# hitfeelee/rtm3d

Measured on AMD Instinct MI355X. Metric: images_per_sec, higher is better.
Workload: dtype fp16

## Files before the change

rtm3d_amd/csrc/common.h:

```cpp
#pragma once
#include <hip/hip_runtime.h>
#include <stdint.h>
#include <stddef.h>

typedef _Float16 f16;
typedef _Float16 f16x8 __attribute__((ext_vector_type(8)));
typedef _Float16 f16x4 __attribute__((ext_vector_type(4)));
typedef _Float16 f16x2 __attribute__((ext_vector_type(2)));
typedef float f32x4 __attribute__((ext_vector_type(4)));
typedef uint32_t u32x4 __attribute__((ext_vector_type(4)));

__device__ __forceinline__ int div_small_q(int m, int d, float rcp_d) {
    const int q = (int)((float)m * rcp_d);
    const int r = m - q * d;
    return q + (r >= d ? 1 : 0) - (r < 0 ? 1 : 0);
}


#define RT_DMA16(gptr, lds_byte_addr) \
    asm volatile("s_mov_b32 m0, %1\n\ts_nop 0\n\tglobal_load_lds_dwordx4 %0, off" : : "v"(gptr), "s"(lds_byte_addr) : "memory", "m0")
#define RT_DMA16_NT(gptr, lds_byte_addr) \
    asm volatile("s_mov_b32 m0, %1\n\ts_nop 0\n\tglobal_load_lds_dwordx4 %0, off nt" : : "v"(gptr), "s"(lds_byte_addr) : "memory", "m0")
static __device__ __forceinline__ const void* rt_uniform_ptr(const void* p) {
    const unsigned long long v = (unsigned long long)p;
    const unsigned lo = (unsigned)__builtin_amdgcn_readfirstlane((int)(unsigned)v), hi = (unsigned)__builtin_amdgcn_readfirstlane((int)(unsigned)(v >> 32));
    return (const void*)(((unsigned long long)hi << 32) | lo);
}
#define RT_DMA16_SBASE(voff_bytes, sbase, lds_byte_addr) \
    asm volatile("s_mov_b32 m0, %2\n\ts_nop 0\n\tglobal_load_lds_dwordx4 %0, %1" : : "v"(voff_bytes), "s"(rt_uniform_ptr(sbase)), "s"(lds_byte_addr) : "memory", "m0")

#define RT_DMA16_SBASE_LANES(voff_bytes, sbase, lds_byte_addr, lanemask) \
    { unsigned long long rt_exec_; \
      asm volatile("s_mov_b64 %0, exec\n\ts_and_b64 exec, exec, %4\n\ts_mov_b32 m0, %3\n\ts_nop 0\n\tglobal_load_lds_dwordx4 %1, %2\n\ts_mov_b64 exec, %0" \
                   : "=&s"(rt_exec_) : "v"(voff_bytes), "s"(rt_uniform_ptr(sbase)), "s"(lds_byte_addr), "s"(lanemask) : "memory", "m0", "scc"); }
#define RT_DMA16_SBASE_NT(voff_bytes, sbase, lds_byte_addr) \
    asm volatile("s_mov_b32 m0, %2\n\ts_nop 0\n\tglobal_load_lds_dwordx4 %0, %1 nt" : : "v"(voff_bytes), "s"(rt_uniform_ptr(sbase)), "s"(lds_byte_addr) : "memory", "m0")

#define RT_MAX_GROUPS 4
#define RT_MAX_TAPS 80

struct ConvGroupArgs {
    int in_coff, out_coff, res_coff;
    int out_oy, out_ox;
    uint32_t w_off;
    int bias_off;
    int tap_off[RT_MAX_TAPS];
};

struct ConvKArgs {
    const f16* in;
    const f16* wgt;
    const float* bias;
    const f16* res;
    void* out;
    int M, HmWm, Wm;
    int in_Hp, in_Wp, in_C, in_stride, in_P;
    int out_Hp, out_Wp, out_C, out_scale, out_P;
    int res_Hp, res_Wp, res_C, res_P;
    int cin, cout, ksteps, cpt;
    int ntaps;
    int relu, MT, NT;
    int out_H, out_W;
    float* slab;
    int ksplit;
    int deep;
    f16* s2d;
    int s_Hp, s_Wp, s_C, s_P, s_coff;
    int in_s2d;
    ConvGroupArgs g[RT_MAX_GROUPS];
};

struct HaloTaps { unsigned long long taps[RT_MAX_GROUPS]; };

struct PoolKArgs {
    const f16* in; f16* out;
    int B, Ho, Wo, C8;
    int in_Hp, in_Wp, in_C, in_P, in_coff;
    int out_Hp, out_Wp, out_C, out_P, out_coff;
    int ksize, stride, pad;
};

struct SoftmaxKArgs {
    const f16* z_in; f16* z_out;
    const f16* u[3];
    int n_u;
    int B, H, W, C;
    int z_Hp, z_Wp, z_C, z_P;
    int zi_Hp, zi_Wp, zi_C, zi_P;
    int u_Hp[3], u_Wp[3], u_C[3], u_P[3];
    float* partial;
    float* stats;
    int chunks, rows_per_chunk;
    int apply_chunks, apply_rows, xsplit, seg_w;
    int partial_chunks;
};

__device__ __forceinline__ int xcd_contiguous_index(int b, int n) {
#ifdef RT_TIMING_NO_XCD_ORDER
    return b;
#endif
    const int q = n >> 3, r = n & 7, xcd = b & 7, k = b >> 3;
    return xcd * q + (xcd < r ? xcd : r) + k;
}

struct HeadOutArgs {
    const f16* in;
    const f16* wgt;
    const float* bias;
    float* out[4];
    int cout[4];
    int nheads;
    int B, H, W;
    int in_Hp, in_Wp, in_C, in_P;
    int tiles_x, tiles_y, tile_rows;
};

struct StemFusedArgs {
    const f16* x4;
    const float* x_nchw;
    f16* out;
    const f16* w_base;
    const f16* w_l0;
    const f16* w_l1;
    const float* b_base;
    const float* b_l0;
    const float* b_l1;
    int B, H, W;
    int x_Hp, x_Wp, x_P;
    int o_Hp, o_Wp, o_C, o_P, o_coff;
    int tiles_x, tiles_y;
};

struct Conv32S2Args {
    const f16* in;
    f16* out_conv;
    f16* out_proj;
    const f16* w_conv;
    const f16* w_proj;
    const float* b_conv;
    const float* b_proj;
    int B, Ho, Wo;
    int in_Hp, in_Wp, in_C, in_P, in_coff;
    int oc_Hp, oc_Wp, oc_C, oc_P, oc_coff;
    int op_Hp, op_Wp, op_C, op_P, op_coff;
};

struct RootKArgs {
    const f16* w;
    const float* bias;
    f16* out;
    int o_Hp, o_Wp, o_C, o_P, o_coff;
    f16* pool;
    int p_Hp, p_Wp, p_C, p_P, p_coff;
    f16* s2d;
    int s_Hp, s_Wp, s_C, s_P, s_coff;
    int relu;
};

struct PatchMaskArgs {
    f16* base;
    const int32_t* yx;
    int n_slots, S, C, img_H, img_W, origin;
};

struct ConvMx8Args {
    const uint8_t* in; const uint8_t* in_s;
    const uint8_t* wgt;
    const uint8_t* wsc;
    const float* bias;
    void* out; uint8_t* out_s;
    int M, HmWm, Wm;
    int in_Hp, in_Wp, in_C, in_P;
    int out_Hp, out_Wp, out_C, out_P;
    int cin, cout, ntaps, cpt, ksteps;
    int relu, out_fp16, MT, NT;
    int in_coff[RT_MAX_GROUPS], out_coff[RT_MAX_GROUPS];
    int tap_pix[RT_MAX_TAPS];
};
struct QuantMx8Args {
    const f16* in;
    uint8_t* out;
    uint8_t* out_s;
    int B, H, W;
    int in_Hp, in_Wp, in_C, in_P, in_coff;
    int out_Hp, out_Wp, out_C, out_P, out_coff;
    int nblk;
};

struct PersistentGrid { int grid, single; };
inline PersistentGrid persistent_grid(int total, int cu_count) { return {cu_count < total ? cu_count : total, total <= cu_count ? 1 : 0}; }

hipError_t launch_patch_mask(const PatchMaskArgs& a, hipStream_t s);
hipError_t launch_conv32s2_fused(const Conv32S2Args& a, int cu_count, unsigned int* ticket_ctr, hipStream_t s);
hipError_t launch_stem_fused(const StemFusedArgs& a, hipStream_t s);
hipError_t launch_conv_headout(const HeadOutArgs& a, hipStream_t s);
hipError_t launch_conv_mfma(const ConvKArgs& a, int bn_tile, int groups, int epi_nchw, hipStream_t s);
hipError_t launch_conv_mfma_deep(const ConvKArgs& a, int bn_tile, int groups, unsigned int* tile_ctr, hipStream_t s);
hipError_t launch_conv_mfma256(const ConvKArgs& a, int groups, unsigned int* tile_ctr, float* stat_out, hipStream_t s);
enum Conv256Route { C256_ONE_TILE, C256_PERSISTENT, C256_HALO, C256_LATTICE };
Conv256Route conv_mfma256_route(const ConvKArgs& a, int groups, HaloTaps* ht);
void conv_mfma256_permute_weights(const f16* src, f16* dst, size_t n_ktiles);
bool conv64_halo_supported(const ConvKArgs& a, int groups);
hipError_t launch_conv64_halo(const ConvKArgs& a, int cu_count, unsigned int* ticket_ctr, hipStream_t s);
hipError_t launch_conv64_root(const ConvKArgs& a, const RootKArgs& r, int cu_count, unsigned int* ticket_ctr, hipStream_t s);
bool conv64s2_halo_supported(const ConvKArgs& a, int groups);
hipError_t launch_conv64s2_halo(const ConvKArgs& a, int cu_count, unsigned int* ticket_ctr, hipStream_t s);
bool conv128_halo_supported(const ConvKArgs& a, int groups);
hipError_t launch_conv128_halo(const ConvKArgs& a, int cu_count, unsigned int* ticket_ctr, hipStream_t s);
hipError_t launch_conv_smallc(const ConvKArgs& a, hipStream_t s);
bool conv_smallc_supported(int cin, int cout, int ntaps);
hipError_t launch_nchw_to_nhwc4(const float* in, f16* out, int B, int H, int W, int Hp, int Wp, int P, hipStream_t s);
hipError_t launch_maxpool(const PoolKArgs& a, hipStream_t s);
hipError_t launch_softmax_fuse(const SoftmaxKArgs& a, hipStream_t s);
hipError_t launch_quant_mx8(const QuantMx8Args& a, hipStream_t s);
hipError_t launch_conv_mx8(const ConvMx8Args& a, int groups, hipStream_t s);
```

rtm3d_amd/csrc/conv_mfma256.hip:

```cpp
#include <string.h>
#include "common.h"

#define LDS_AS __attribute__((address_space(3)))
#define GLB_AS __attribute__((address_space(1)))

void conv_mfma256_permute_weights(const f16* src, f16* dst, size_t n_ktiles) {
    for (size_t k = 0; k < n_ktiles; ++k)
        for (int rd = 0; rd < 256; ++rd) {
            const int j = rd >> 7, wc = (rd >> 5) & 3, c = (rd >> 4) & 1, frow = rd & 15;
            const int rs = wc * 64 + frow * 4 + j * 2 + c;
            for (int pos = 0; pos < 8; ++pos) {
                const int chunk = pos ^ (rd & 7);
                memcpy(dst + (k * 256 + rd) * 64 + pos * 8, src + (k * 256 + rs) * 64 + (chunk ^ (rs & 7)) * 8, 16);
            }
        }
}

#define HALF_ELEMS (128 * 64)
#define BUF_ELEMS (4 * HALF_ELEMS)
#define SLOT_XA 0
#define SLOT_XB 1
#define SLOT_WA 2
#define SLOT_WB 3

__device__ __forceinline__ void c256_next_pixel(int& n, int& y, int& x, bool live, int Wm, int Hm) {
    const bool wx = x + 1 == Wm, wy = wx && y + 1 == Hm;
    const int x1 = wx ? 0 : x + 1, y1 = wy ? 0 : (wx ? y + 1 : y), n1 = wy ? n + 1 : n;
    x = live ? x1 : x; y = live ? y1 : y; n = live ? n1 : n;
}

template <int RES>
__global__ __launch_bounds__(512) void conv_mfma256_kernel(const ConvKArgs a) {
    __shared__ __attribute__((aligned(16))) f16 lds[2 * BUF_ELEMS + HALF_ELEMS];
    const int tid = threadIdx.x;
    const int lane = tid & 63;
    const int wave = __builtin_amdgcn_readfirstlane(tid >> 6);
    const int wp = wave & 1, wc = wave >> 1;

    const int bid = blockIdx.x;
    const int xcd = bid & 7, jb = bid >> 3;
    const int chunk = (a.MT + 7) >> 3;
    const int ntile = jb % a.NT;
    const int mtile = xcd * chunk + jb / a.NT;
    if (mtile >= a.MT) return;
    const ConvGroupArgs& g = a.g[blockIdx.y];
    const int T = a.ksteps;

    uint32_t xoff[2][2];
    {
        const int rr = tid >> 3, cs = tid & 7;
#pragma unroll
        for (int h = 0; h < 2; ++h)
#pragma unroll
            for (int i = 0; i < 2; ++i) {
                int m = mtile * 256 + h * 128 + i * 64 + rr;
                m = m < a.M ? m : a.M - 1;
                const int n = m / a.HmWm, rem = m - n * a.HmWm;
                const int y = rem / a.Wm, x = rem - y * a.Wm;
                const uint32_t pix = (uint32_t)((n * a.in_Hp + y * a.in_stride + a.in_P) * a.in_Wp + x * a.in_stride + a.in_P);
                xoff[h][i] = pix * (uint32_t)a.in_C + (uint32_t)g.in_coff + (uint32_t)((cs ^ (rr & 7)) * 8);
            }
    }
    const f16* wbase = a.wgt + g.w_off + (size_t)ntile * T * (256 * 64);
    f16* const dummy = lds + 2 * BUF_ELEMS;

    auto stage = [&](int slot, int kt) {
        const bool live = kt < T;
        const int k = live ? kt : T - 1;
        f16* dst = live ? (lds + (k & 1) * BUF_ELEMS + slot * HALF_ELEMS) : dummy;
        if (slot < 2) {
            const int tap = k / a.cpt, q = k - tap * a.cpt;
            const int koff = g.tap_off[tap] + q * 64;
#pragma unroll
            for (int i = 0; i < 2; ++i) {
                const f16* src = a.in + (size_t)xoff[slot][i] + (ptrdiff_t)koff;
                __builtin_amdgcn_global_load_lds((const GLB_AS void*)src, (LDS_AS void*)(dst + (i * 512 + wave * 64) * 8), 16, 0, 0);
            }
        } else {
            const f16* ws = wbase + (size_t)k * (256 * 64) + (slot - 2) * HALF_ELEMS;
#pragma unroll
            for (int i = 0; i < 2; ++i)
                __builtin_amdgcn_global_load_lds((const GLB_AS void*)(ws + (i * 512 + tid) * 8),
                                                 (LDS_AS void*)(dst + (i * 512 + wave * 64) * 8), 16, 0, 0);
        }
    };

    f32x4 acc[2][2][2][4];
#pragma unroll
    for (int i = 0; i < 2; ++i)
#pragma unroll
        for (int j = 0; j < 2; ++j)
#pragma unroll
            for (int c = 0; c < 2; ++c)
#pragma unroll
                for (int p = 0; p < 4; ++p) acc[i][j][c][p] = (f32x4){0.f, 0.f, 0.f, 0.f};

    const int frow = lane & 15, fk = lane >> 4;
    const int sw0 = ((0 * 4 + fk) ^ (frow & 7)) * 8, sw1 = ((1 * 4 + fk) ^ (frow & 7)) * 8;
    const int xrow = (wp * 64 + frow) * 64;
    const int wrow = (wc * 32 + frow) * 64;

    stage(SLOT_XA, 0); stage(SLOT_WA, 0); stage(SLOT_WB, 0); stage(SLOT_XB, 0);
    stage(SLOT_XA, 1); stage(SLOT_WA, 1);
    asm volatile("s_waitcnt vmcnt(4)" ::: "memory");
    __builtin_amdgcn_s_barrier();
    if (wave >= 4) __builtin_amdgcn_s_barrier();

    f16x8 xf[4][2], wa[2][2], wb[2][2];

#define LOAD_X(slot_base)                                                                   \
    _Pragma("unroll") for (int p = 0; p < 4; ++p) {                                         \
        xf[p][0] = *(const f16x8*)((slot_base) + xrow + p * 1024 + sw0);                    \
        xf[p][1] = *(const f16x8*)((slot_base) + xrow + p * 1024 + sw1);                    \
    }
#define LOAD_W(dstf, slot_base)                                                             \
    _Pragma("unroll") for (int c = 0; c < 2; ++c) {                                         \
        dstf[c][0] = *(const f16x8*)((slot_base) + wrow + c * 1024 + sw0);                  \
        dstf[c][1] = *(const f16x8*)((slot_base) + wrow + c * 1024 + sw1);                  \
    }
#define SEG_SYNC()                                                                          \
    asm volatile("s_waitcnt vmcnt(8)" ::: "memory");                                        \
    __builtin_amdgcn_sched_barrier(0);                                                      \
    __builtin_amdgcn_s_barrier();                                                           \
    __builtin_amdgcn_sched_barrier(0);
#define MMA(i, j, wfrag)                                                                    \
    __builtin_amdgcn_s_setprio(1);                                                          \
    _Pragma("unroll") for (int kk = 0; kk < 2; ++kk)                                        \
        _Pragma("unroll") for (int c = 0; c < 2; ++c)                                       \
            _Pragma("unroll") for (int p = 0; p < 4; ++p)                                   \
                acc[i][j][c][p] = __builtin_amdgcn_mfma_f32_16x16x32_f16(xf[p][kk], wfrag[c][kk], acc[i][j][c][p], 0, 0, 0); \
    __builtin_amdgcn_s_setprio(0);                                                          \
    __builtin_amdgcn_sched_barrier(0);                                                      \
    __builtin_amdgcn_s_barrier();                                                           \
    __builtin_amdgcn_sched_barrier(0);

    for (int t = 0; t < T; ++t) {
        const f16* buf = lds + (t & 1) * BUF_ELEMS;
        LOAD_X(buf + SLOT_XA * HALF_ELEMS)
        LOAD_W(wa, buf + SLOT_WA * HALF_ELEMS)
        stage(SLOT_WB, t + 1);
        SEG_SYNC()
        MMA(0, 0, wa)
        LOAD_W(wb, buf + SLOT_WB * HALF_ELEMS)
        stage(SLOT_XB, t + 1);
        SEG_SYNC()
        MMA(0, 1, wb)
        LOAD_X(buf + SLOT_XB * HALF_ELEMS)
        stage(SLOT_XA, t + 2);
        SEG_SYNC()
        MMA(1, 1, wb)
        stage(SLOT_WA, t + 2);
        SEG_SYNC()
        MMA(1, 0, wa)
    }
    if (wave < 4) __builtin_amdgcn_s_barrier();

    const f32x4 bv = *(const f32x4*)(a.bias + g.bias_off + ntile * 256 + wc * 64 + frow * 4);
    const float lo = a.relu ? 0.f : -__builtin_inff();
    const int cbase = ntile * 256 + wc * 64 + frow * 4;
    const int Hm = a.HmWm / a.Wm;
#pragma unroll
    for (int i = 0; i < 2; ++i) {
        size_t opix[4][4];
        f16x4 rv[4][4];
#pragma unroll
        for (int p = 0; p < 4; ++p) {
            const int m0 = mtile * 256 + i * 128 + wp * 64 + p * 16 + fk * 4;
            const int m = m0 < a.M ? m0 : a.M - 1;
            int n = m / a.HmWm;
            const int rem = m - n * a.HmWm;
            int y = rem / a.Wm, x = rem - y * a.Wm;
#pragma unroll
            for (int e = 0; e < 4; ++e) {
                if (e) c256_next_pixel(n, y, x, m0 + e < a.M, a.Wm, Hm);
                const int oy = y * a.out_scale + g.out_oy, ox = x * a.out_scale + g.out_ox;
                opix[p][e] = ((size_t)(n * a.out_Hp + oy + a.out_P) * a.out_Wp + ox + a.out_P) * a.out_C + g.out_coff + cbase;
                if (RES) rv[p][e] = *(const f16x4*)(a.res + ((size_t)(n * a.res_Hp + oy + a.res_P) * a.res_Wp + ox + a.res_P) * a.res_C + g.res_coff + cbase);
            }
        }
#pragma unroll
        for (int p = 0; p < 4; ++p)
#pragma unroll
            for (int e = 0; e < 4; ++e) {
                f32x4 v = {acc[i][0][0][p][e], acc[i][0][1][p][e], acc[i][1][0][p][e], acc[i][1][1][p][e]};
                v += bv;
                if (RES) {
                    const f16x4 r = rv[p][e];
                    v[0] += (float)r[0]; v[1] += (float)r[1]; v[2] += (float)r[2]; v[3] += (float)r[3];
                }
                const f16x4 h = {(f16)fmaxf(v[0], lo), (f16)fmaxf(v[1], lo), (f16)fmaxf(v[2], lo), (f16)fmaxf(v[3], lo)};
                *(f16x4*)((f16*)a.out + opix[p][e]) = h;
            }
    }
}

#define CONV256_MAX_BIAS 2048
#define DMA16 RT_DMA16
#define DMA16_NT RT_DMA16_NT
#define DMA16_SBASE RT_DMA16_SBASE
#define DMA16_SBASE_NT RT_DMA16_SBASE_NT
#define LDS_F16X8(byte_addr) (*(const LDS_AS f16x8*)(uintptr_t)(byte_addr))
#define LOAD_X_N(SLOT)                                                                      \
    _Pragma("unroll") for (int p = 0; p < 4; ++p) {                                         \
        xf[p][0] = LDS_F16X8(xaddr0 + (SLOT) * HALF_ELEMS * 2 + p * 2048);                  \
        xf[p][1] = LDS_F16X8(xaddr1 + (SLOT) * HALF_ELEMS * 2 + p * 2048);                  \
    }
#define LOAD_W_N(dstf, SLOT)                                                                \
    _Pragma("unroll") for (int c = 0; c < 2; ++c) {                                         \
        dstf[c][0] = LDS_F16X8(waddr0 + (SLOT) * HALF_ELEMS * 2 + c * 2048);                \
        dstf[c][1] = LDS_F16X8(waddr1 + (SLOT) * HALF_ELEMS * 2 + c * 2048);                \
    }
#ifdef C256_T_NOVM
#define SEG_SYNC_N(VM)                                                                      \
    asm volatile("s_waitcnt lgkmcnt(0)" ::: "memory");                                      \
    __builtin_amdgcn_sched_barrier(0);                                                      \
    __builtin_amdgcn_s_barrier();                                                           \
    __builtin_amdgcn_sched_barrier(0);
#else
#define SEG_SYNC_N(VM)                                                                      \
    asm volatile("s_waitcnt vmcnt(" #VM ") lgkmcnt(0)" ::: "memory");                       \
    __builtin_amdgcn_sched_barrier(0);                                                      \
    __builtin_amdgcn_s_barrier();                                                           \
    __builtin_amdgcn_sched_barrier(0);
#endif
#define MMA_N(i, j, wfrag, FIRST, TAILBAR)                                                  \
    __builtin_amdgcn_s_setprio(1);                                                          \
    _Pragma("unroll") for (int kk = 0; kk < 2; ++kk)                                        \
        _Pragma("unroll") for (int c = 0; c < 2; ++c)                                       \
            _Pragma("unroll") for (int p = 0; p < 4; ++p)                                   \
                acc[i][j][c][p] = __builtin_amdgcn_mfma_f32_16x16x32_f16(xf[p][kk], wfrag[c][kk], acc[i][j][c][p], 0, 0, 0); \
    __builtin_amdgcn_s_setprio(0);                                                          \
    __builtin_amdgcn_sched_barrier(0);                                                      \
    if (TAILBAR) __builtin_amdgcn_s_barrier();                                              \
    __builtin_amdgcn_sched_barrier(0);
#ifdef C256_STAMPS
#define C256_STAMP_KT 20
#define C256_STAMP_N 20
#define STAMP(k) if ((wave & 3) == 0 && stamp_tile == 1 && t < C256_STAMP_KT) { unsigned long long ts_; \
        asm volatile("s_memtime %0\n\ts_waitcnt lgkmcnt(0)" : "=s"(ts_) :: "memory"); if (lane == 0) lds_stamp[wave >> 2][t][k] = ts_; }
#define TSTAMP(k) if ((wave & 3) == 0 && stamp_tile < 4) { unsigned long long ts_; \
        asm volatile("s_memtime %0\n\ts_waitcnt lgkmcnt(0)" : "=s"(ts_) :: "memory"); if (lane == 0) lds_tstamp[wave >> 2][stamp_tile][k] = ts_; }
#else
#define STAMP(k)
#define TSTAMP(k)
#endif
#ifdef C256_STAMPS
#define SEG_SYNC_S(VM, K0)                                                                  \
    STAMP((K0) + 0)                                                                         \
    asm volatile("s_waitcnt vmcnt(" #VM ") lgkmcnt(0)" ::: "memory");                       \
    STAMP((K0) + 1)                                                                         \
    __builtin_amdgcn_sched_barrier(0);                                                      \
    __builtin_amdgcn_s_barrier();                                                           \
    __builtin_amdgcn_sched_barrier(0);                                                      \
    STAMP((K0) + 2)
#define MMA_S(i, j, wfrag, FIRST, TAILBAR, K0)                                              \
    __builtin_amdgcn_s_setprio(1);                                                          \
    _Pragma("unroll") for (int kk = 0; kk < 2; ++kk)                                        \
        _Pragma("unroll") for (int c = 0; c < 2; ++c)                                       \
            _Pragma("unroll") for (int p = 0; p < 4; ++p)                                   \
                acc[i][j][c][p] = __builtin_amdgcn_mfma_f32_16x16x32_f16(xf[p][kk], wfrag[c][kk], acc[i][j][c][p], 0, 0, 0); \
    __builtin_amdgcn_s_setprio(0);                                                          \
    __builtin_amdgcn_sched_barrier(0);                                                      \
    STAMP((K0) + 3)                                                                         \
    if (TAILBAR) __builtin_amdgcn_s_barrier();                                              \
    __builtin_amdgcn_sched_barrier(0);                                                      \
    STAMP((K0) + 4)
#else
#define SEG_SYNC_S(VM, K0) SEG_SYNC_N(VM)
#define MMA_S(i, j, wfrag, FIRST, TAILBAR, K0) MMA_N(i, j, wfrag, FIRST, TAILBAR)
#endif
#if !defined(C256_WB_IN_P4)
#define STAGE_WB_P1 stage_w1(SLOT_WB, 0, t + 1, sp ^ 1);
#define STAGE_WB_P2 stage_w1(SLOT_WB, 1, t + 1, sp ^ 1);
#define STAGE_WB_P4
#define VM1_8 5
#define VM1_40 37
#else
#define STAGE_WB_P1
#define STAGE_WB_P2
#define STAGE_WB_P4 stage(SLOT_WB, t + 2, sp, 0);
#define VM1_8 8
#define VM1_40 40
#endif
#define OPA_SET(SP)                                                                         \
    {                                                                                       \
        const uint32_t bufb_ = lds_base + (uint32_t)(SP) * (BUF_ELEMS * 2);                 \
        opa[0] = bufb_ + xrow_b0; opa[1] = bufb_ + xrow_b1; opa[2] = bufb_ + wrow_b0; opa[3] = bufb_ + wrow_b1; \
    }
#define STEP_N(VM, VM1, FIRST, LAST)                                                          \
    {                                                                                       \
         \
        const uint32_t xaddr0 = opa[0], xaddr1 = opa[1], waddr0 = opa[2], waddr1 = opa[3];  \
        LOAD_X_N(SLOT_XA)                                                                   \
        LOAD_W_N(wa, SLOT_WA)                                                               \
        STAGE_WB_P1                                                                         \
        SEG_SYNC_S(VM1, 0)                                                                  \
        MMA_S(0, 0, wa, FIRST, 1, 0)                                                        \
        LOAD_W_N(wb, SLOT_WB)                                                               \
        stage(SLOT_XB, t + 1, sp ^ 1, koff1);                                               \
        STAGE_WB_P2                                                                         \
        SEG_SYNC_S(VM, 5)                                                                   \
        MMA_S(0, 1, wb, FIRST, 1, 5)                                                        \
        LOAD_X_N(SLOT_XB)                                                                   \
        stage(SLOT_XA, t + 2, sp, koff2);                                                   \
        SEG_SYNC_S(VM, 10)                                                                  \
        MMA_S(1, 1, wb, FIRST, 1, 10)                                                       \
         \
              \
        int kchan3;                                                                         \
        int kraw3 = koff_parts(t + 3, kchan3);                                              \
        stage(SLOT_WA, t + 2, sp, 0);                                                       \
        OPA_SET(sp ^ 1)                                                                     \
        asm volatile("" : "+v"(opa[0]), "+v"(opa[1]), "+v"(opa[2]), "+v"(opa[3]));          \
        STAGE_WB_P4                                                                         \
        SEG_SYNC_S(VM, 15)                                                                  \
        asm volatile("" : "+s"(kraw3));            \
        const int koff3 = kraw3 + kchan3;                                                   \
        MMA_S(1, 0, wa, FIRST, !(LAST), 15)                                                 \
        koff1 = koff2; koff2 = koff3;                                                       \
        sp ^= 1;                                                                            \
    }

template <int RES, int XNT>
__global__ __launch_bounds__(512) void conv_mfma256_persistent_kernel(const ConvKArgs a, const int groups, const int nbias, unsigned int* tile_ctr, const int one_list) {
    __shared__ __attribute__((aligned(16))) f16 lds[2 * BUF_ELEMS + HALF_ELEMS];
    __shared__ __attribute__((aligned(16))) float lds_bias[CONV256_MAX_BIAS + 4];
#ifdef C256_STAMPS
    __shared__ unsigned long long lds_stamp[2][C256_STAMP_KT][C256_STAMP_N];
    __shared__ unsigned long long lds_tstamp[2][4][4];
    int stamp_tile = 0;
#endif
    const int tid = threadIdx.x;
    const int lane = tid & 63;
    const int wave = __builtin_amdgcn_readfirstlane(tid >> 6);
    const int wp = wave & 1, wc = wave >> 1;
    const int T = a.ksteps;
    for (int i = tid; i < nbias; i += 512) lds_bias[i] = a.bias[i];
    __syncthreads();

    const int xcd = one_list ? 0 : blockIdx.x & 7, per_xcd = one_list ? gridDim.x : gridDim.x >> 3;
    const int chunk = one_list ? a.MT : (a.MT + 7) >> 3;
    int mt_here = a.MT - xcd * chunk;
    mt_here = mt_here < 0 ? 0 : (mt_here > chunk ? chunk : mt_here);
    const int jbs = mt_here * a.NT;
    const int vtotal = jbs * groups;
    int* const lds_ticket = (int*)(lds_bias + CONV256_MAX_BIAS);
    const int last_draw = vtotal + per_xcd - 1;
    if (tid == 0) {
        const int t0 = (int)atomicAdd(&tile_ctr[xcd], 1u);
        if (t0 == last_draw) tile_ctr[xcd] = 0u;
        lds_ticket[0] = t0;
    }
    __syncthreads();
    const int v = __builtin_amdgcn_readfirstlane(lds_ticket[0]);
    if (v >= vtotal) return;

    const uint32_t lds_base = (uint32_t)(uintptr_t)(LDS_AS f16*)lds;
    const int rr = tid >> 3, cs = tid & 7;
    const float rcp_hw = 1.0f / (float)a.HmWm, rcp_w = 1.0f / (float)a.Wm;
    uint32_t xo_c[2][2], xo_n[2][2];
    const f16 *wb_c, *wb_n;
    int gi_c, gi_n, mt_c, mt_n, nt_c, nt_n;
    auto locate = [&](int vv, uint32_t (&xo)[2][2], const f16*& wb, int& gi, int& mt, int& nt) {
        gi = vv / jbs;
        const int jb = vv - gi * jbs;
        const int q = jb / a.NT;
        nt = jb - q * a.NT;
        mt = xcd * chunk + q;
        const ConvGroupArgs& g = a.g[gi];
#pragma unroll
        for (int h = 0; h < 2; ++h)
#pragma unroll
            for (int i = 0; i < 2; ++i) {
                int m = mt * 256 + h * 128 + i * 64 + rr;
                m = m < a.M ? m : a.M - 1;
                const int n = div_small_q(m, a.HmWm, rcp_hw), rem = m - n * a.HmWm;
                const int y = div_small_q(rem, a.Wm, rcp_w), x = rem - y * a.Wm;
                const uint32_t pix = (uint32_t)((n * a.in_Hp + y * a.in_stride + a.in_P) * a.in_Wp + x * a.in_stride + a.in_P);
                xo[h][i] = (pix * (uint32_t)a.in_C + (uint32_t)g.in_coff + (uint32_t)((cs ^ (rr & 7)) * 8)) * 2u;
            }
#ifdef C256_T_WSAME
        wb = a.wgt + g.w_off;
#else
        wb = a.wgt + g.w_off + (size_t)nt * T * (256 * 64);
#endif
    };
    bool live_n;
    locate(v, xo_c, wb_c, gi_c, mt_c, nt_c);
    xo_n[0][0] = xo_c[0][0]; xo_n[0][1] = xo_c[0][1]; xo_n[1][0] = xo_c[1][0]; xo_n[1][1] = xo_c[1][1];
    wb_n = wb_c; gi_n = gi_c; mt_n = mt_c; nt_n = nt_c; live_n = false;

    auto koff_parts = [&](int kpos, int& chan) -> int {
        const bool in_cur = kpos < T;
        const int k = in_cur ? kpos : kpos - T;
        const int tap = k / a.cpt;
        chan = (k - tap * a.cpt) * 64;
        return a.g[in_cur ? gi_c : gi_n].tap_off[tap];
    };
    auto koff_of = [&](int kpos) -> int { int c; const int r = koff_parts(kpos, c); return r + c; };
    const uint32_t wvoff = (uint32_t)tid * 16u;
    auto stage_w1 = [&](int slot, int i, int kpos, int par) {
        const bool in_cur = kpos < T;
        const int k = in_cur ? kpos : kpos - T;
        const uint32_t dst0 = lds_base + (uint32_t)((in_cur || live_n) ? par * BUF_ELEMS + slot * HALF_ELEMS : 2 * BUF_ELEMS) * 2u;
        const f16* ws = (in_cur ? wb_c : wb_n) + (size_t)k * (256 * 64) + (slot - 2) * HALF_ELEMS;
        DMA16_SBASE(wvoff, ws + i * 512 * 8, __builtin_amdgcn_readfirstlane(dst0 + (uint32_t)((i * 512 + wave * 64) * 16)));
    };
    auto stage = [&](int slot, int kpos, int par, int koff) {
        const bool in_cur = kpos < T;
        const int k = in_cur ? kpos : kpos - T;
        const uint32_t dst0 = lds_base + (uint32_t)((in_cur || live_n) ? par * BUF_ELEMS + slot * HALF_ELEMS : 2 * BUF_ELEMS) * 2u;
        if (slot < 2) {
#ifdef C256_T_NOX
            return;
#endif
            const f16* xbase = a.in + (ptrdiff_t)koff;
#pragma unroll
            for (int i = 0; i < 2; ++i) {
                const uint32_t xo = in_cur ? xo_c[slot][i] : xo_n[slot][i];
                if (XNT) DMA16_SBASE_NT(xo, xbase, __builtin_amdgcn_readfirstlane(dst0 + (uint32_t)((i * 512 + wave * 64) * 16)));
                else DMA16_SBASE(xo, xbase, __builtin_amdgcn_readfirstlane(dst0 + (uint32_t)((i * 512 + wave * 64) * 16)));
            }
        } else {
#ifdef C256_T_NOW
            return;
#endif
            const f16* ws = (in_cur ? wb_c : wb_n) + (size_t)k * (256 * 64) + (slot - 2) * HALF_ELEMS;
#pragma unroll
            for (int i = 0; i < 2; ++i)
                DMA16_SBASE(wvoff, ws + i * 512 * 8, __builtin_amdgcn_readfirstlane(dst0 + (uint32_t)((i * 512 + wave * 64) * 16)));
        }
    };

    f32x4 acc[2][2][2][4];
    const int frow = lane & 15, fk = lane >> 4;
    const int sw0 = ((0 * 4 + fk) ^ (frow & 7)) * 8, sw1 = ((1 * 4 + fk) ^ (frow & 7)) * 8;
    const uint32_t xrow_b0 = (uint32_t)(((wp * 64 + frow) * 64 + sw0) * 2), xrow_b1 = (uint32_t)(((wp * 64 + frow) * 64 + sw1) * 2);
    const uint32_t wrow_b0 = (uint32_t)(((wc * 32 + frow) * 64 + sw0) * 2), wrow_b1 = (uint32_t)(((wc * 32 + frow) * 64 + sw1) * 2);
    const int Hm = a.HmWm / a.Wm;
    const f16 lo = a.relu ? (f16)0.f : (f16)(-__builtin_inff());
    const f16x4 lo4 = {lo, lo, lo, lo};

    stage(SLOT_XA, 0, 0, koff_of(0)); stage(SLOT_WA, 0, 0, 0); stage(SLOT_WB, 0, 0, 0); stage(SLOT_XB, 0, 0, koff_of(0));
    stage(SLOT_XA, 1, 1, koff_of(1)); stage(SLOT_WA, 1, 1, 0);
#ifndef C256_WB_IN_P4
    asm volatile("s_waitcnt vmcnt(4)" ::: "memory");
#else
    stage(SLOT_WB, 1, 1, 0);
    asm volatile("s_waitcnt vmcnt(6)" ::: "memory");
#endif
    if (tid == 0) {
        const int t1 = (int)atomicAdd(&tile_ctr[xcd], 1u);
        if (t1 == last_draw) tile_ctr[xcd] = 0u;
        lds_ticket[1] = t1;
    }
    asm volatile("s_waitcnt lgkmcnt(0)" ::: "memory");
    __builtin_amdgcn_s_barrier();
    int vnext = __builtin_amdgcn_readfirstlane(lds_ticket[1]);
    if (wave >= 4) __builtin_amdgcn_s_barrier();

    f16x8 xf[4][2], wa[2][2], wb[2][2];
    int sp = 0;
    int tpar = 0;
    int koff1 = koff_of(1), koff2 = koff_of(2);
    bool first_tile = true;
    uint32_t opa[4];
    OPA_SET(0)

    for (;;) {
        int ticket = vnext;
        const bool draw = vnext < vtotal;
        if (wave == 0 && draw) {
            const unsigned inc = 1u, off = (unsigned)xcd * 4u;
            unsigned long long saved_exec;
            asm volatile("s_mov_b64 %1, exec\n\ts_mov_b64 exec, 1\n\tglobal_atomic_add %0, %2, %3, %4 sc0\n\ts_mov_b64 exec, %1"
                         : "=&v"(ticket), "=&s"(saved_exec) : "v"(off), "v"(inc), "s"(tile_ctr) : "memory");
        }
        {
            f32x4 b4 = *(const f32x4*)__builtin_assume_aligned(lds_bias + a.g[gi_c].bias_off + nt_c * 256 + wc * 64 + frow * 4, 16);
            asm volatile("" : "+v"(b4));
#pragma unroll
            for (int j = 0; j < 2; ++j)
#pragma unroll
                for (int c = 0; c < 2; ++c) {
                    const float b = b4[j * 2 + c];
#pragma unroll
                    for (int i = 0; i < 2; ++i)
#pragma unroll
                        for (int p = 0; p < 4; ++p) acc[i][j][c][p] = (f32x4){b, b, b, b};
                }
        }
        int t = 0;
        TSTAMP(0)
        if (first_tile) STEP_N(8, VM1_8, 1, 0) else STEP_N(40, VM1_40, 1, 0)
        first_tile = false;
        if (wave == 0) {
            asm volatile("s_waitcnt vmcnt(8)" : "+v"(ticket) : : "memory");
            if (lane == 0) {
                lds_ticket[tpar] = ticket;
                if (draw && ticket == last_draw) tile_ctr[xcd] = 0u;
            }
        }
        live_n = draw;
        if (live_n) locate(vnext, xo_n, wb_n, gi_n, mt_n, nt_n);
        for (t = 1; t < T - 1; ++t) STEP_N(8, VM1_8, 0, 0)
        STEP_N(8, VM1_8, 0, 1)
        if (wave < 4) __builtin_amdgcn_s_barrier();
        TSTAMP(1)

        {
            const ConvGroupArgs& g = a.g[gi_c];
            const int cbase = nt_c * 256 + wc * 64 + frow * 4;
#pragma unroll
            for (int i = 0; i < 2; ++i) {
                size_t opix[4][4];
                f16x4 rv[4][4];
#pragma unroll
                for (int p = 0; p < 4; ++p) {
                    const int m0 = mt_c * 256 + i * 128 + wp * 64 + p * 16 + fk * 4;
                    const int m = m0 < a.M ? m0 : a.M - 1;
                    int n = div_small_q(m, a.HmWm, rcp_hw);
                    const int rem = m - n * a.HmWm;
                    int y = div_small_q(rem, a.Wm, rcp_w), x = rem - y * a.Wm;
#pragma unroll
                    for (int e = 0; e < 4; ++e) {
                        if (e) c256_next_pixel(n, y, x, m0 + e < a.M, a.Wm, Hm);
                        const int oy = y * a.out_scale + g.out_oy, ox = x * a.out_scale + g.out_ox;
                        opix[p][e] = ((size_t)(n * a.out_Hp + oy + a.out_P) * a.out_Wp + ox + a.out_P) * a.out_C + g.out_coff + cbase;
                        if (RES) rv[p][e] = *(const f16x4*)(a.res + ((size_t)(n * a.res_Hp + oy + a.res_P) * a.res_Wp + ox + a.res_P) * a.res_C + g.res_coff + cbase);
                    }
                }
#pragma unroll
                for (int p = 0; p < 4; ++p)
#pragma unroll
                    for (int e = 0; e < 4; ++e) {
                        f32x4 vv = {acc[i][0][0][p][e], acc[i][0][1][p][e], acc[i][1][0][p][e], acc[i][1][1][p][e]};
                        if (RES) {
                            const f16x4 r = rv[p][e];
                            vv[0] += (float)r[0]; vv[1] += (float)r[1]; vv[2] += (float)r[2]; vv[3] += (float)r[3];
                        }
                        f16x4 h = {(f16)vv[0], (f16)vv[1], (f16)vv[2], (f16)vv[3]};
                        h = __builtin_elementwise_max(h, lo4);
                        *(f16x4*)((f16*)a.out + opix[p][e]) = h;
                    }
            }
        }
        TSTAMP(2)
        if (wave >= 4) __builtin_amdgcn_s_barrier();
        TSTAMP(3)
#ifdef C256_STAMPS
        ++stamp_tile;
#endif
        if (!live_n) break;
        vnext = __builtin_amdgcn_readfirstlane(lds_ticket[tpar]);
        tpar ^= 1;
        xo_c[0][0] = xo_n[0][0]; xo_c[0][1] = xo_n[0][1]; xo_c[1][0] = xo_n[1][0]; xo_c[1][1] = xo_n[1][1];
        wb_c = wb_n; gi_c = gi_n; mt_c = mt_n; nt_c = nt_n;
    }
    if (wave < 4) __builtin_amdgcn_s_barrier();
#ifdef C256_STAMPS
    if ((blockIdx.x == 0 || blockIdx.x == 101) && (wave & 3) == 0) {
        asm volatile("s_waitcnt vmcnt(0) lgkmcnt(0)" ::: "memory");
        unsigned long long* dst = (unsigned long long*)(tile_ctr + 1024) + (blockIdx.x ? 1 : 0) * 1024 + (wave >> 2) * 512;
        for (int i = lane; i < C256_STAMP_KT * C256_STAMP_N; i += 64) dst[i] = (&lds_stamp[wave >> 2][0][0])[i];
        if (lane < 16) dst[C256_STAMP_KT * C256_STAMP_N + lane] = (&lds_tstamp[wave >> 2][0][0])[lane];
        if (lane == 16) dst[C256_STAMP_KT * C256_STAMP_N + 16] = (unsigned long long)T;
    }
#endif
}

bool conv_mfma256_halo_supported(const ConvKArgs& a, int groups, HaloTaps* ht);
hipError_t launch_conv_mfma256_halo(const ConvKArgs& a, const HaloTaps& ht, int groups, int nbias, int cu_count, unsigned int* tile_ctr, float* stat_out, hipStream_t s);
int conv_mfma256_lattice_dilation(const ConvKArgs& a, int groups);
hipError_t launch_conv_mfma256_lattice(const ConvKArgs& a, int groups, int nbias, int cu_count, unsigned int* tile_ctr, hipStream_t s);

static int device_cu_count() {
    static int n = 0;
    if (!n) {
        int dev = 0;
        hipDeviceProp_t prop;
        if (hipGetDevice(&dev) != hipSuccess || hipGetDeviceProperties(&prop, dev) != hipSuccess) return 256;
        n = prop.multiProcessorCount;
    }
    return n;
}

static int conv256_nbias(const ConvKArgs& a, int groups) {
    int nbias = 0;
    for (int g = 0; g < groups; ++g) nbias = a.g[g].bias_off + a.cout > nbias ? a.g[g].bias_off + a.cout : nbias;
    return (nbias + 255) / 256 * 256;
}

Conv256Route conv_mfma256_route(const ConvKArgs& a, int groups, HaloTaps* ht) {
    const int nbias = conv256_nbias(a, groups);
    const unsigned long long in_bytes = (unsigned long long)(a.M / a.HmWm) * a.in_Hp * a.in_Wp * a.in_C * 2ull;
    if (a.ksteps < 4 || nbias > CONV256_MAX_BIAS || in_bytes >= (1ull << 32)) return C256_ONE_TILE;
    HaloTaps scratch;
    if (!ht) ht = &scratch;
#ifdef C256_T_NOHALO9
    if (a.ntaps == 9) {} else
#endif
    if (!a.res && (a.ntaps == 9 || a.ntaps == 4) && nbias <= 1024 && conv_mfma256_halo_supported(a, groups, ht)) return C256_HALO;
#ifndef C256_T_NOLATTICE
    if (nbias <= 1024 && conv_mfma256_lattice_dilation(a, groups) != 0) return C256_LATTICE;
#endif
    return C256_PERSISTENT;
}

hipError_t launch_conv_mfma256(const ConvKArgs& a, int groups, unsigned int* tile_ctr, float* stat_out, hipStream_t s) {
    dim3 block(512, 1, 1);
    HaloTaps ht;
    const Conv256Route route = conv_mfma256_route(a, groups, &ht);
    if (stat_out && route != C256_HALO) return hipErrorInvalidValue;
    if (route != C256_ONE_TILE && !tile_ctr) return hipErrorInvalidValue;
    const int nbias = conv256_nbias(a, groups);
    if (route == C256_HALO) return launch_conv_mfma256_halo(a, ht, groups, nbias, device_cu_count(), tile_ctr, stat_out, s);
    if (route == C256_LATTICE) return launch_conv_mfma256_lattice(a, groups, nbias, device_cu_count(), tile_ctr, s);
    if (route == C256_PERSISTENT) {
        const int per_xcd = device_cu_count() / 8;
        const int one_list = (long long)a.MT * a.NT * groups <= device_cu_count() ? 1 : 0;
        dim3 grid(per_xcd * 8, 1, 1);
        const bool x_once = !a.res && a.ntaps == 1 && a.NT == 1 && a.in_stride == 1;
        if (a.res) hipLaunchKernelGGL((conv_mfma256_persistent_kernel<1, 0>), grid, block, 0, s, a, groups, nbias, tile_ctr, one_list);
        else if (x_once) hipLaunchKernelGGL((conv_mfma256_persistent_kernel<0, 1>), grid, block, 0, s, a, groups, nbias, tile_ctr, one_list);
        else hipLaunchKernelGGL((conv_mfma256_persistent_kernel<0, 0>), grid, block, 0, s, a, groups, nbias, tile_ctr, one_list);
        return hipGetLastError();
    }
    const int mt8 = (a.MT + 7) / 8 * 8;
    dim3 grid(mt8 * a.NT, groups, 1);
    if (a.res) hipLaunchKernelGGL((conv_mfma256_kernel<1>), grid, block, 0, s, a);
    else hipLaunchKernelGGL((conv_mfma256_kernel<0>), grid, block, 0, s, a);
    return hipGetLastError();
}
```

rtm3d_amd/csrc/pool_softmax.hip:

```cpp
#include "common.h"

__global__ __launch_bounds__(256) void maxpool_kernel(const PoolKArgs a) {
    const int idx = blockIdx.x * 256 + threadIdx.x;
    const int total = a.B * a.Ho * a.Wo * a.C8;
    if (idx >= total) return;
    const int c8 = idx % a.C8;
    int p = idx / a.C8;
    const int ox = p % a.Wo; p /= a.Wo;
    const int oy = p % a.Ho;
    const int n = p / a.Ho;
    f16x8 m;
    bool first = true;
    if (a.ksize == 0) {
        const f16* ip = a.in + ((size_t)(n * a.in_Hp + oy + a.in_P) * a.in_Wp + ox + a.in_P) * a.in_C + a.in_coff + c8 * 8;
        m = *(const f16x8*)ip;
#pragma unroll
        for (int ph = 1; ph < 4; ++ph) {
            const f16x8 v = *(const f16x8*)(ip + ph * a.C8 * 8);
#pragma unroll
            for (int e = 0; e < 8; ++e) m[e] = v[e] > m[e] ? v[e] : m[e];
        }
        first = false;
    }
    for (int ky = 0; ky < a.ksize; ++ky)
        for (int kx = 0; kx < a.ksize; ++kx) {
            const int iy = oy * a.stride - a.pad + ky + a.in_P, ix = ox * a.stride - a.pad + kx + a.in_P;
            const f16x8 v = *(const f16x8*)(a.in + ((size_t)(n * a.in_Hp + iy) * a.in_Wp + ix) * a.in_C + a.in_coff + c8 * 8);
            if (first) { m = v; first = false; }
            else {
#pragma unroll
                for (int e = 0; e < 8; ++e) m[e] = v[e] > m[e] ? v[e] : m[e];
            }
        }
    *(f16x8*)(a.out + ((size_t)(n * a.out_Hp + oy + a.out_P) * a.out_Wp + ox + a.out_P) * a.out_C + a.out_coff + c8 * 8) = m;
}

hipError_t launch_maxpool(const PoolKArgs& a, hipStream_t s) {
    const int total = a.B * a.Ho * a.Wo * a.C8;
    hipLaunchKernelGGL(maxpool_kernel, dim3((total + 255) / 256), dim3(256), 0, s, a);
    return hipGetLastError();
}

__global__ __launch_bounds__(256) void softmax_reduce_kernel(const SoftmaxKArgs a) {
    const int chunk = blockIdx.x, n = blockIdx.y, ui = blockIdx.z;
    const int lane = threadIdx.x & 63, wave = threadIdx.x >> 6;
    const int cg = lane & 31, slot = wave * 2 + (lane >> 5);
    const f16* u = a.u[ui];
    const int Hp = a.u_Hp[ui], Wp = a.u_Wp[ui], C = a.u_C[ui], P = a.u_P[ui];
    float m[8], s[8];
#pragma unroll
    for (int e = 0; e < 8; ++e) { m[e] = -INFINITY; s[e] = 0.f; }
    const int y0 = chunk * a.rows_per_chunk;
    const int y1 = min(y0 + a.rows_per_chunk, a.H);
    for (int y = y0; y < y1; ++y) {
        const f16* row = u + ((size_t)(n * Hp + y + P) * Wp + P) * C + cg * 8;
        for (int x = slot; x < a.W; x += 32) {
            f16x8 v[4];
#pragma unroll
            for (int k = 0; k < 4; ++k) {
                const int xx = x + 8 * k < a.W ? x + 8 * k : x;
                v[k] = *(const f16x8*)(row + (size_t)xx * C);
            }
#pragma unroll
            for (int e = 0; e < 8; ++e) {
                float f[4];
#pragma unroll
                for (int k = 0; k < 4; ++k) f[k] = (x + 8 * k < a.W) ? (float)v[k][e] : -INFINITY;
                const float mn = fmaxf(fmaxf(fmaxf(f[0], f[1]), fmaxf(f[2], f[3])), m[e]);
                s[e] = s[e] * __expf(m[e] - mn) + ((__expf(f[0] - mn) + __expf(f[1] - mn)) + (__expf(f[2] - mn) + __expf(f[3] - mn)));
                m[e] = mn;
            }
        }
    }
    __shared__ float sm[8][256], ss[8][256];
#pragma unroll
    for (int e = 0; e < 8; ++e) { sm[slot][cg * 8 + e] = m[e]; ss[slot][cg * 8 + e] = s[e]; }
    __syncthreads();
    const int c = threadIdx.x;
    float M = -INFINITY;
#pragma unroll
    for (int w = 0; w < 8; ++w) M = fmaxf(M, sm[w][c]);
    float S = 0.f;
#pragma unroll
    for (int w = 0; w < 8; ++w) S += (sm[w][c] == -INFINITY) ? 0.f : ss[w][c] * __expf(sm[w][c] - M);
    float* out = a.partial + ((((size_t)ui * a.B + n) * a.chunks + chunk) * a.C + c) * 2;
    out[0] = M; out[1] = S;
}

__global__ __launch_bounds__(1024) void softmax_combine_kernel(const SoftmaxKArgs a) {
    const int n = blockIdx.x, ui = blockIdx.y, cl = threadIdx.x & 63, c = blockIdx.z * 64 + cl, part = threadIdx.x >> 6;
    const int chunks = a.partial_chunks > 0 ? a.partial_chunks : a.chunks;
    const float2* p = (const float2*)a.partial + ((size_t)ui * a.B + n) * chunks * a.C + c;
    float m = -INFINITY, sum = 0.f;
    for (int k = part; k < chunks; k += 16) {
        const float2 v = p[(size_t)k * a.C];
        if (v.x != -INFINITY) {
            const float mn = fmaxf(m, v.x);
            sum = sum * __expf(m - mn) + v.y * __expf(v.x - mn);
            m = mn;
        }
    }
    __shared__ float sm[16][64], ss[16][64];
    sm[part][cl] = m; ss[part][cl] = sum;
    __syncthreads();
    if (part == 0) {
        float mm = sm[0][cl];
#pragma unroll
        for (int w = 1; w < 16; ++w) mm = fmaxf(mm, sm[w][cl]);
        float t = 0.f;
#pragma unroll
        for (int w = 0; w < 16; ++w) t += (sm[w][cl] == -INFINITY) ? 0.f : ss[w][cl] * __expf(sm[w][cl] - mm);
        float* o = a.stats + (((size_t)ui * a.B + n) * a.C + c) * 2;
        o[0] = mm; o[1] = 1.f / t;
    }
}

template <int NU>
__global__ __launch_bounds__(256) void softmax_apply_kernel(const SoftmaxKArgs a) {
    const int chunk = blockIdx.x, n = blockIdx.y;
    const int rchunk = chunk / a.xsplit, xseg = chunk - rchunk * a.xsplit;
    const int x0 = xseg * a.seg_w, x1 = min(x0 + a.seg_w, a.W);
    const int lane = threadIdx.x & 63, wave = threadIdx.x >> 6;
    const int cg = lane & 31, slot = wave * 2 + (lane >> 5);
    float M[NU][8], invS[NU][8];
#pragma unroll
    for (int ui = 0; ui < NU; ++ui) {
        const float* st = a.stats + (((size_t)ui * a.B + n) * a.C + cg * 8) * 2;
#pragma unroll
        for (int e = 0; e < 8; ++e) { M[ui][e] = st[2 * e]; invS[ui][e] = st[2 * e + 1]; }
    }
    const int y0 = rchunk * a.apply_rows;
    const int y1 = min(y0 + a.apply_rows, a.H);
    for (int y = y0; y < y1; ++y) {
        const size_t zrow = ((size_t)(n * a.z_Hp + y + a.z_P) * a.z_Wp + a.z_P) * a.z_C + cg * 8;
        const size_t zirow = ((size_t)(n * a.zi_Hp + y + a.zi_P) * a.zi_Wp + a.zi_P) * a.zi_C + cg * 8;
        size_t urow[NU];
#pragma unroll
        for (int ui = 0; ui < NU; ++ui) urow[ui] = ((size_t)(n * a.u_Hp[ui] + y + a.u_P[ui]) * a.u_Wp[ui] + a.u_P[ui]) * a.u_C[ui] + cg * 8;
        for (int x = x0 + slot; x < x1; x += 16) {
            f16x8 zi[2], v[2][NU];
#pragma unroll
            for (int k = 0; k < 2; ++k) {
                const int xx = x + 8 * k < x1 ? x + 8 * k : x;
                zi[k] = __builtin_nontemporal_load((const f16x8*)(a.z_in + zirow + (size_t)xx * a.zi_C));
#pragma unroll
                for (int ui = 0; ui < NU; ++ui) v[k][ui] = __builtin_nontemporal_load((const f16x8*)(a.u[ui] + urow[ui] + (size_t)xx * a.u_C[ui]));
            }
#pragma unroll
            for (int k = 0; k < 2; ++k) {
                if (x + 8 * k >= x1) break;
                f16x8 o;
#pragma unroll
                for (int e = 0; e < 8; ++e) {
                    float acc = (float)zi[k][e];
#pragma unroll
                    for (int ui = 0; ui < NU; ++ui) {
                        const float f = (float)v[k][ui][e];
                        acc += f * (__expf(f - M[ui][e]) * invS[ui][e]);
                    }
                    o[e] = (f16)acc;
                }
                *(f16x8*)(a.z_out + zrow + (size_t)(x + 8 * k) * a.z_C) = o;
            }
        }
    }
}

hipError_t launch_softmax_fuse(const SoftmaxKArgs& a, hipStream_t s) {
    if (a.C != 256 || a.n_u < 1 || a.n_u > 3 || a.xsplit < 1 || a.seg_w < 1 || a.apply_rows < 1) return hipErrorInvalidValue;
    if (a.partial_chunks <= 0) hipLaunchKernelGGL(softmax_reduce_kernel, dim3(a.chunks, a.B, a.n_u), dim3(256), 0, s, a);
    hipLaunchKernelGGL(softmax_combine_kernel, dim3(a.B, a.n_u, a.C / 64), dim3(1024), 0, s, a);
    if (a.n_u == 3) hipLaunchKernelGGL(softmax_apply_kernel<3>, dim3(a.apply_chunks, a.B, 1), dim3(256), 0, s, a);
    else if (a.n_u == 2) hipLaunchKernelGGL(softmax_apply_kernel<2>, dim3(a.apply_chunks, a.B, 1), dim3(256), 0, s, a);
    else hipLaunchKernelGGL(softmax_apply_kernel<1>, dim3(a.apply_chunks, a.B, 1), dim3(256), 0, s, a);
    return hipGetLastError();
}
```

rtm3d_amd/csrc/runtime.hip:

```cpp
#include <math.h>
#include <stdarg.h>
#include <stdio.h>
#include <string.h>
#include <string>
#include <vector>

#include "common.h"
#include "../../include/rtm3d_hip.h"

static thread_local char g_err[512] = "";
void rt_set_error(const char* fmt, ...) {
    va_list ap;
    va_start(ap, fmt);
    vsnprintf(g_err, sizeof(g_err), fmt, ap);
    va_end(ap);
}
#define RT_FAIL(...) do { rt_set_error(__VA_ARGS__); return 1; } while (0)
#define RT_HIP(expr) do { hipError_t e_ = (expr); if (e_ != hipSuccess) { rt_set_error("%s: %s", #expr, hipGetErrorString(e_)); return 1; } } while (0)

struct Tensor {
    int B, H, W, C, P, Hp, Wp;
    f16* alloc;
    f16* base;
    size_t elems;
};

struct MxTensor {
    int B, H, W, C, P, Hp, Wp;
    uint8_t* alloc;
    uint8_t* base;
    uint8_t* s_alloc;
    uint8_t* s_base;
    size_t elems;
};

enum OpKind { OP_CONV_MFMA, OP_CONV_MFMA256, OP_CONV64_HALO, OP_CONV64_ROOT, OP_CONV64S2_HALO, OP_CONV128_HALO, OP_STEM_FUSED, OP_CONV32S2_FUSED, OP_CONV_SMALLC, OP_INPUT4, OP_HEADOUT, OP_MAXPOOL, OP_SOFTMAX, OP_PATCH_MASK, OP_QUANT_MX8, OP_CONV_MX8 };

struct Op {
    OpKind kind;
    std::string name;
    double flops, bytes;
    ConvKArgs conv; int groups, bn_tile, epi_nchw, out_slot;
    int ticket_slot = -1;
    float* stat_out = nullptr;
    Tensor input4;
    bool input4_unread = false;
    PoolKArgs pool;
    SoftmaxKArgs sm;
    HeadOutArgs ho;
    StemFusedArgs sf;
    Conv32S2Args c32;
    PatchMaskArgs pm;
    RootKArgs root;
    QuantMx8Args qm;
    ConvMx8Args cm;
};

struct rtm3d_ctx {
    int device;
    int n_cus = 256;
    std::vector<Tensor> tensors;
    std::vector<struct MxTensor> mx8;
    std::vector<void*> blobs;
    std::vector<size_t> blob_bytes;
    std::vector<Op> ops;
    std::vector<void*> extra;
    float* stat_buf = nullptr;
    int stat_chunks = 0, stat_B = 0;
    int stat_tensor[3] = {-1, -1, -1};
    unsigned int* tile_ctr = nullptr;
    int ticket_slots_used = 0;
    float* slab = nullptr;
    size_t slab_floats = 0;
    int probe_op = -1;
    std::vector<hipEvent_t> probe_ev;
    int probe_count = 0;
    int graph_mode = 0;
    hipStream_t capture_stream = nullptr;
    hipStream_t last_stream = nullptr;
    bool has_last = false;
    hipEvent_t done_ev = nullptr;
    struct GraphEntry { const void* key[5]; hipGraph_t graph; hipGraphExec_t exec; unsigned long long last_use; };
    std::vector<GraphEntry> graphs;
    unsigned long long graph_clock = 0, graph_hits = 0, graph_captures = 0, graph_refused = 0;
    int test_memset_in_replay = 0;
    int n_marks = 0;
    int mark_op[8];
    hipEvent_t mark_ev[9];
    void* engine = nullptr;
    void (*engine_free)(void*) = nullptr;
};

void rt_ctx_attach_engine(rtm3d_ctx* ctx, void* engine, void (*engine_free)(void*)) {
    ctx->engine = engine;
    ctx->engine_free = engine_free;
}
void* rt_ctx_engine(rtm3d_ctx* ctx) { return ctx ? ctx->engine : nullptr; }

static const int PROBE_RING = 64;
static const int TICKET_SLOTS = 56;
static const int SPLIT_CTRS = 256;
static const size_t TILE_CTR_WORDS = 8 + TICKET_SLOTS + SPLIT_CTRS;
static const size_t DEBUG_WORD0 = 1024;
static const size_t DEBUG_WORDS = 16384;

static int ensure_tile_ctr(rtm3d_ctx* ctx) {
    if (ctx->tile_ctr) return 0;
    RT_HIP(hipMalloc((void**)&ctx->tile_ctr, (DEBUG_WORD0 + DEBUG_WORDS) * sizeof(unsigned int)));
    RT_HIP(hipMemset(ctx->tile_ctr, 0, (DEBUG_WORD0 + DEBUG_WORDS) * sizeof(unsigned int)));
    ctx->extra.push_back(ctx->tile_ctr);
    return 0;
}
static unsigned int* ticket_ctr(rtm3d_ctx* ctx, const Op& op) { return ctx->tile_ctr + 8 + op.ticket_slot; }
static unsigned int* split_ctrs(rtm3d_ctx* ctx) { return ctx->tile_ctr + 8 + TICKET_SLOTS; }

static int claim_ticket(rtm3d_ctx* ctx, Op& op, const char* what) {
    if (ctx->ticket_slots_used >= TICKET_SLOTS) RT_FAIL("%s: out of ticket counters", what);
    if (ensure_tile_ctr(ctx)) return 1;
    op.ticket_slot = ctx->ticket_slots_used++;
    return 0;
}

static bool slice_ok(int coff, int n, int C) { return coff >= 0 && coff + n <= C && coff % 8 == 0; }

extern "C" const char* rtm3d_last_error(void) { return g_err; }
extern "C" int rtm3d_abi_version(void) { return RTM3D_ABI_VERSION; }

extern "C" int rtm3d_ctx_create(int device, rtm3d_ctx** out) {
    if (!out) RT_FAIL("ctx_create: null out");
    RT_HIP(hipSetDevice(device));
    int xccs = 0, cus = 0;
    RT_HIP(hipDeviceGetAttribute(&cus, hipDeviceAttributeMultiprocessorCount, device));
    if (hipDeviceGetAttribute(&xccs, hipDeviceAttributeNumberOfXccs, device) != hipSuccess) xccs = 0;
    if ((xccs != 0 && xccs != 8) || cus < 8 || (cus % 8) != 0)
        RT_FAIL("ctx_create: device %d reports %d XCCs / %d CUs; librtm3d_hip is built for the 8-XCD (SPX) MI355X", device, xccs, cus);
    rtm3d_ctx* c = new rtm3d_ctx();
    c->device = device;
    c->n_cus = cus;
    *out = c;
    return 0;
}

extern "C" void rtm3d_ctx_destroy(rtm3d_ctx* ctx) {
    if (!ctx) return;
    for (auto& t : ctx->tensors) (void)hipFree(t.alloc);
    for (auto& t : ctx->mx8) { (void)hipFree(t.alloc); (void)hipFree(t.s_alloc); }
    for (auto p : ctx->blobs) (void)hipFree(p);
    for (auto p : ctx->extra) (void)hipFree(p);
    for (auto e : ctx->probe_ev) (void)hipEventDestroy(e);
    for (auto& ge : ctx->graphs) { (void)hipGraphExecDestroy(ge.exec); (void)hipGraphDestroy(ge.graph); }
    if (ctx->capture_stream) (void)hipStreamDestroy(ctx->capture_stream);
    if (ctx->done_ev) (void)hipEventDestroy(ctx->done_ev);
    if (ctx->engine_free) ctx->engine_free(ctx->engine);
    delete ctx;
}

static const size_t GUARD = 4096;

extern "C" int rtm3d_tensor_create(rtm3d_ctx* ctx, int B, int H, int W, int C, int pad, int* id) {
    if (!ctx || !id) RT_FAIL("tensor_create: null argument");
    if (B <= 0 || H <= 0 || W <= 0 || C <= 0 || pad < 0 || (C % 4) != 0) RT_FAIL("tensor_create: bad shape B=%d H=%d W=%d C=%d pad=%d (C must be a multiple of 4)", B, H, W, C, pad);
    Tensor t;
    t.B = B; t.H = H; t.W = W; t.C = C; t.P = pad; t.Hp = H + 2 * pad; t.Wp = W + 2 * pad;
    t.elems = (size_t)B * t.Hp * t.Wp * C;
    if (t.elems >= ((size_t)1 << 32) - 2 * GUARD) RT_FAIL("tensor_create: %zu elements exceed the 32-bit offset range of the kernels", t.elems);
    const size_t bytes = (t.elems + 2 * GUARD) * sizeof(f16);
    RT_HIP(hipMalloc((void**)&t.alloc, bytes));
    RT_HIP(hipMemset(t.alloc, 0, bytes));
    t.base = t.alloc + GUARD;
    ctx->tensors.push_back(t);
    *id = (int)ctx->tensors.size() - 1;
    return 0;
}

static Tensor* get_tensor(rtm3d_ctx* ctx, int id) {
    if (id < 0 || id >= (int)ctx->tensors.size()) return nullptr;
    return &ctx->tensors[id];
}

extern "C" int rtm3d_tensor_download(rtm3d_ctx* ctx, int id, int c0, int C, float* h_nchw) {
    Tensor* t = ctx ? get_tensor(ctx, id) : nullptr;
    if (!t || !h_nchw || c0 < 0 || C <= 0 || c0 + C > t->C) RT_FAIL("tensor_download: bad arguments");
    std::vector<f16> host(t->elems);
    RT_HIP(hipDeviceSynchronize());
    RT_HIP(hipMemcpy(host.data(), t->base, t->elems * sizeof(f16), hipMemcpyDeviceToHost));
    for (int n = 0; n < t->B; ++n)
        for (int c = 0; c < C; ++c)
            for (int y = 0; y < t->H; ++y)
                for (int x = 0; x < t->W; ++x)
                    h_nchw[(((size_t)n * C + c) * t->H + y) * t->W + x] =
                        (float)host[(((size_t)n * t->Hp + y + t->P) * t->Wp + x + t->P) * t->C + c0 + c];
    return 0;
}

extern "C" int rtm3d_tensor_upload(rtm3d_ctx* ctx, int id, int c0, int C, const float* h_nchw) {
    Tensor* t = ctx ? get_tensor(ctx, id) : nullptr;
    if (!t || !h_nchw || c0 < 0 || C <= 0 || c0 + C > t->C) RT_FAIL("tensor_upload: bad arguments");
    std::vector<f16> host(t->elems);
    RT_HIP(hipDeviceSynchronize());
    RT_HIP(hipMemcpy(host.data(), t->base, t->elems * sizeof(f16), hipMemcpyDeviceToHost));
    for (int n = 0; n < t->B; ++n)
        for (int c = 0; c < C; ++c)
            for (int y = 0; y < t->H; ++y)
                for (int x = 0; x < t->W; ++x)
                    host[(((size_t)n * t->Hp + y + t->P) * t->Wp + x + t->P) * t->C + c0 + c] =
                        (f16)h_nchw[(((size_t)n * C + c) * t->H + y) * t->W + x];
    RT_HIP(hipMemcpy(t->base, host.data(), t->elems * sizeof(f16), hipMemcpyHostToDevice));
    return 0;
}

extern "C" int rtm3d_blob_create(rtm3d_ctx* ctx, const void* h_data, size_t bytes, int* id) {
    if (!ctx || !h_data || !id || bytes == 0) RT_FAIL("blob_create: bad arguments");
    void* p = nullptr;
    RT_HIP(hipMalloc(&p, bytes + 256));
    RT_HIP(hipMemset(p, 0, bytes + 256));
    RT_HIP(hipMemcpy(p, h_data, bytes, hipMemcpyHostToDevice));
    ctx->blobs.push_back(p);
    ctx->blob_bytes.push_back(bytes);
    *id = (int)ctx->blobs.size() - 1;
    return 0;
}

extern "C" int rtm3d_tensor_info(rtm3d_ctx* ctx, int id, void** d_base, int* B, int* H, int* W, int* C, int* border) {
    Tensor* t = ctx ? get_tensor(ctx, id) : nullptr;
    if (!t) RT_FAIL("tensor_info: bad tensor %d", id);
    if (d_base) *d_base = t->base;
    if (B) *B = t->B;
    if (H) *H = t->H;
    if (W) *W = t->W;
    if (C) *C = t->C;
    if (border) *border = t->P;
    return 0;
}

static void* get_blob(rtm3d_ctx* ctx, int id, size_t* bytes);
extern "C" int rtm3d_blob_address(rtm3d_ctx* ctx, int id, void** d_ptr, size_t* bytes) {
    void* p = ctx ? get_blob(ctx, id, bytes) : nullptr;
    if (!p || !d_ptr) RT_FAIL("blob_address: bad blob %d", id);
    *d_ptr = p;
    return 0;
}

static void* get_blob(rtm3d_ctx* ctx, int id, size_t* bytes) {
    if (id < 0 || id >= (int)ctx->blobs.size()) return nullptr;
    if (bytes) *bytes = ctx->blob_bytes[id];
    return ctx->blobs[id];
}

static int admit_mfma128(rtm3d_ctx* ctx, const rtm3d_conv_desc* d, size_t wbytes, size_t bbytes, Op& op) {
    ConvKArgs& a = op.conv;
    const int BN = d->bn_tile;
    if (BN != 16 && BN != 32 && BN != 64 && BN != 128) RT_FAIL("op_conv: bn_tile must be 16/32/64/128");
    if (d->cin % 64) RT_FAIL("op_conv(mfma): cin=%d is not a multiple of 64", d->cin);
    if (!d->out_nchw_f32 && (d->cout % BN)) RT_FAIL("op_conv(mfma): cout=%d is not a multiple of the tile %d", d->cout, BN);
    if (d->out_nchw_f32 && a.res) RT_FAIL("op_conv(mfma): the NCHW fp32 epilogue adds no residual");
    const int cout_pad = (d->cout + BN - 1) / BN * BN;
    a.cpt = d->cin / 64; a.ksteps = d->ntaps * a.cpt;
    a.MT = (a.M + 127) / 128; a.NT = cout_pad / BN;
    const size_t per_group = (size_t)cout_pad * a.ksteps * 64;
    if (wbytes != per_group * d->groups * sizeof(f16)) RT_FAIL("op_conv(mfma): packed weight blob has %zu bytes, expected %zu", wbytes, per_group * d->groups * sizeof(f16));
    if (bbytes != (size_t)cout_pad * d->groups * sizeof(float)) RT_FAIL("op_conv(mfma): bias blob has %zu bytes, expected %zu", bbytes, (size_t)cout_pad * d->groups * sizeof(float));
    for (int g = 0; g < d->groups; ++g) { a.g[g].w_off = (uint32_t)(per_group * g); a.g[g].bias_off = cout_pad * g; }
    op.kind = OP_CONV_MFMA; op.bn_tile = BN;
    op.name = d->ntaps == 1 ? "conv1x1_mfma" : (d->ntaps == 4 ? "deconv4x4_phase_mfma" : "conv3x3_mfma");
    if (d->out_nchw_f32 || (BN != 64 && BN != 128)) return 0;
    const long long wgs = (long long)a.MT * a.NT * d->groups;
    if (wgs > ctx->n_cus) return 0;
    a.deep = 1;
    op.name += "_deep";
    if (ensure_tile_ctr(ctx)) return 1;
    if (wgs * 2 > ctx->n_cus || wgs > SPLIT_CTRS || a.ksteps < 8) return 0;
    int ks = (int)(ctx->n_cus / wgs);
    if (ks > a.ksteps / 4) ks = a.ksteps / 4;
    if (ks > 16) ks = 16;
    if (ks < 2) return 0;
    const size_t need = (size_t)ks * wgs * 128 * BN;
    if (need > ctx->slab_floats) {
        float* nslab = nullptr;
        RT_HIP(hipMalloc((void**)&nslab, need * sizeof(float)));
        ctx->extra.push_back(nslab);
        for (auto& prev : ctx->ops) if (prev.kind == OP_CONV_MFMA && prev.conv.ksplit > 1) prev.conv.slab = nslab;
        ctx->slab = nslab; ctx->slab_floats = need;
    }
    a.ksplit = ks; a.slab = ctx->slab;
    op.name += "_splitk";
    return 0;
}

static int admit_mfma256(rtm3d_ctx* ctx, const rtm3d_conv_desc* d, size_t wbytes, size_t bbytes, Op& op) {
    ConvKArgs& a = op.conv;
    if (d->cin % 64 || d->cout % 256 || d->out_nchw_f32) RT_FAIL("op_conv(mfma256): needs cin %% 64 == 0, cout %% 256 == 0, NHWC output (cin=%d cout=%d)", d->cin, d->cout);
    a.cpt = d->cin / 64; a.ksteps = d->ntaps * a.cpt;
    a.MT = (a.M + 255) / 256; a.NT = d->cout / 256;
    const size_t per_group = (size_t)d->cout * a.ksteps * 64;
    if (wbytes != per_group * d->groups * sizeof(f16)) RT_FAIL("op_conv(mfma256): packed weight blob has %zu bytes, expected %zu", wbytes, per_group * d->groups * sizeof(f16));
    if (bbytes != (size_t)d->cout * d->groups * sizeof(float)) RT_FAIL("op_conv(mfma256): bias blob size mismatch");
    for (int g = 0; g < d->groups; ++g) { a.g[g].w_off = (uint32_t)(per_group * g); a.g[g].bias_off = d->cout * g; }
    op.kind = OP_CONV_MFMA256; op.bn_tile = 256;
    if (ensure_tile_ctr(ctx)) return 1;
    {
        std::vector<f16> h_src(wbytes / sizeof(f16)), h_dst(wbytes / sizeof(f16));
        RT_HIP(hipMemcpy(h_src.data(), a.wgt, wbytes, hipMemcpyDeviceToHost));
        conv_mfma256_permute_weights(h_src.data(), h_dst.data(), wbytes / (256 * 64 * sizeof(f16)));
        f16* w_perm = nullptr;
        RT_HIP(hipMalloc((void**)&w_perm, wbytes + 256));
        ctx->extra.push_back(w_perm);
        RT_HIP(hipMemset(w_perm, 0, wbytes + 256));
        RT_HIP(hipMemcpy(w_perm, h_dst.data(), wbytes, hipMemcpyHostToDevice));
        a.wgt = w_perm;
    }
    static const char* const suffix[] = {"_1tile", "", "_halo", "_lattice"};
    op.name = d->ntaps == 1 ? "conv1x1_mfma256" : (d->ntaps == 4 ? "deconv4x4_phase_mfma256" : "conv3x3_mfma256");
    op.name += suffix[conv_mfma256_route(a, d->groups, nullptr)];
    return 0;
}

static int admit_smallc(rtm3d_ctx*, const rtm3d_conv_desc* d, size_t wbytes, size_t bbytes, Op& op) {
    ConvKArgs& a = op.conv;
    if (d->groups != 1) RT_FAIL("op_conv(smallc): groups=%d unsupported (one group)", d->groups);
    if (d->out_nchw_f32) RT_FAIL("op_conv(smallc): NCHW output unsupported");
    if (a.res) RT_FAIL("op_conv(smallc): residual unsupported");
    if (!conv_smallc_supported(d->cin, d->cout, d->ntaps)) RT_FAIL("op_conv(smallc): no kernel for cin=%d cout=%d ntaps=%d", d->cin, d->cout, d->ntaps);
    int S = d->cin == 16 ? 5 : (d->cin == 32 ? d->ntaps : 7);
    if (d->cin == 16 && d->cout == 16 && d->in_stride == 1 && d->out_scale == 1 && wbytes == (size_t)(d->cout / 16) * 6 * 64 * 8 * sizeof(f16)) S = 6;
    if (wbytes != (size_t)(d->cout / 16) * S * 64 * 8 * sizeof(f16)) RT_FAIL("op_conv(smallc): weight blob size mismatch");
    a.ksteps = S;
    if (bbytes != (size_t)d->cout * sizeof(float)) RT_FAIL("op_conv(smallc): bias blob size mismatch");
    if (d->cin == 4 && a.in_P < 4) RT_FAIL("op_conv(smallc): the NHWC4 stem input needs a border of 4");
    if (d->cin == 4 && (a.in_C != 4 || d->in_coff[0] != 0)) RT_FAIL("op_conv(smallc): cin=4 reads a 4-channel NHWC4 tensor (input tensor has %d channels, in_coff=%d)", a.in_C, d->in_coff[0]);
    if (d->cin != 4 && a.in_C % 8) RT_FAIL("op_conv(smallc): 16-byte operand loads are misaligned in an input tensor of %d channels (needs a multiple of 8)", a.in_C);
    if (d->cout != 16 && a.out_C % 8) RT_FAIL("op_conv(smallc): 16-byte stores are misaligned in an output tensor of %d channels (needs a multiple of 8)", a.out_C);
    const int* dy = d->tap_dy[0];
    const int* dx = d->tap_dx[0];
    const bool rows = d->in_stride == 1 && d->out_scale == 1 && d->cout == 16 && (d->cin == 4 || (d->cin == 16 && S == 6));
    if (rows) {
        const int K = d->cin == 4 ? 7 : 3;
        for (int t = 0; t < d->ntaps; ++t)
            if (dy[t] != dy[0] + t / K || dx[t] != dx[0] + t % K)
                RT_FAIL("op_conv(smallc): tap geometry: the vertical-walk kernel needs the dense %dx%d taps in row-major order, dilation 1 (tap %d is (%d,%d), expected (%d,%d))",
                        K, K, t, dy[t], dx[t], dy[0] + t / K, dx[0] + t % K);
    } else if (d->cin == 4) {
        for (int t = 0; t < d->ntaps; ++t)
            if (t % 7 && (dy[t] != dy[t - 1] || dx[t] != dx[t - 1] + 1))
                RT_FAIL("op_conv(smallc): tap geometry: cin=4 needs the 7 taps of a filter row on adjacent pixels (tap %d is (%d,%d) after (%d,%d))",
                        t, dy[t], dx[t], dy[t - 1], dx[t - 1]);
    }
    if (d->cin == 4)
        for (int ky = 0; ky < 7; ++ky)
            if ((d->Wm - 1) * d->in_stride + dx[ky * 7 + 6] + 1 >= a.in_Wp - a.in_P)
                RT_FAIL("op_conv(smallc): the pixel right of tap (%d,%d), read with zero weight, leaves the padded input", dy[ky * 7 + 6], dx[ky * 7 + 6]);
    a.g[0].w_off = 0; a.g[0].bias_off = 0;
    op.kind = OP_CONV_SMALLC;
    op.name = d->cin == 4 ? "stem7x7_regmfma" : "conv_smallc_regmfma";
    return 0;
}

static int admit_c64_halo(rtm3d_ctx* ctx, const rtm3d_conv_desc* d, size_t wbytes, size_t bbytes, Op& op) {
    ConvKArgs& a = op.conv;
    if (d->out_nchw_f32) RT_FAIL("op_conv(conv64): NCHW output unsupported");
    if (!a.out) RT_FAIL("op_conv: writing ONLY the space-to-depth copy needs kernel 0");
    a.cpt = 1; a.ksteps = 9; a.MT = 0; a.NT = 1;
    if (!conv64_halo_supported(a, d->groups)) RT_FAIL("op_conv(conv64): needs one 64->64 3x3 stride-1 conv on a map with W %% 32 == 0, H %% 8 == 0");
    if (wbytes != (size_t)9 * 64 * 64 * sizeof(f16) || bbytes != 64 * sizeof(float)) RT_FAIL("op_conv(conv64): weight/bias blob size mismatch");
    if (claim_ticket(ctx, op, "op_conv(conv64)")) return 1;
    a.g[0].w_off = 0; a.g[0].bias_off = 0;
    op.kind = OP_CONV64_HALO; op.bn_tile = 64;
    op.name = "conv3x3_c64_halo";
    return 0;
}

static int admit_c128_halo(rtm3d_ctx* ctx, const rtm3d_conv_desc* d, size_t wbytes, size_t bbytes, Op& op) {
    ConvKArgs& a = op.conv;
    if (d->out_nchw_f32) RT_FAIL("op_conv(conv128): NCHW output unsupported");
    a.cpt = d->cin / 64; a.ksteps = 9 * a.cpt; a.MT = 0; a.NT = 1;
    if (!conv128_halo_supported(a, d->groups)) RT_FAIL("op_conv(conv128): needs one 3x3 stride-1 conv with cin, cout %% 128 == 0 on a map with W %% 32 == 0, H %% 8 == 0");
    if (d->bn_tile != 128 || wbytes != (size_t)9 * d->cin * d->cout * sizeof(f16) || bbytes != (size_t)d->cout * sizeof(float))
        RT_FAIL("op_conv(conv128): weight/bias blob size mismatch (expects the bn_tile = 128 packing)");
    if (claim_ticket(ctx, op, "op_conv(conv128)")) return 1;
    a.g[0].w_off = 0; a.g[0].bias_off = 0;
    op.kind = OP_CONV128_HALO; op.bn_tile = 128;
    op.name = "conv3x3_c128_halo";
    return 0;
}

static int admit_c64s2_halo(rtm3d_ctx* ctx, const rtm3d_conv_desc* d, size_t wbytes, size_t bbytes, Op& op) {
    ConvKArgs& a = op.conv;
    if (d->in_s2d) {
        if (d->groups != 1) RT_FAIL("op_conv: a space-to-depth INPUT is read by kernel 7 only");
        if (!slice_ok(d->in_coff[0], 4 * d->cin, a.in_C) || a.in_P < 1) RT_FAIL("op_conv: the space-to-depth input needs 4 x cin channels behind in_coff and a border >= 1");
    }
    if (d->out_nchw_f32 || a.res) RT_FAIL("op_conv(conv64s2): NCHW output / residual unsupported");
    a.cpt = 1; a.ksteps = 9; a.MT = 0; a.NT = 1;
    a.in_s2d = d->in_s2d ? 1 : 0;
    if (!conv64s2_halo_supported(a, d->groups)) RT_FAIL("op_conv(conv64s2): needs one 64->128 3x3 stride-2 conv onto a map with W %% 32 == 0, H %% 4 == 0 (input border >= 1)");
    if (wbytes != (size_t)9 * 64 * 128 * sizeof(f16) || bbytes != 128 * sizeof(float)) RT_FAIL("op_conv(conv64s2): weight/bias blob size mismatch");
    if (claim_ticket(ctx, op, "op_conv(conv64s2)")) return 1;
    a.g[0].w_off = 0; a.g[0].bias_off = 0;
    op.kind = OP_CONV64S2_HALO; op.bn_tile = 128;
    op.name = "conv3x3s2_c64_halo";
    return 0;
}

extern "C" int rtm3d_op_conv(rtm3d_ctx* ctx, const rtm3d_conv_desc* d) {
    if (!ctx || !d) RT_FAIL("op_conv: null argument");
    Tensor* in = get_tensor(ctx, d->in_tensor);
    if (d->s2d_tensor < 0) RT_FAIL("op_conv: s2d_tensor = %d (tensor id + 1, 0 = none)", d->s2d_tensor);
    const int s2d_id = d->s2d_tensor - 1;
    const bool s2d_only = !d->out_nchw_f32 && d->out_tensor < 0 && s2d_id >= 0;
    Tensor* out = (d->out_nchw_f32 || s2d_only) ? nullptr : get_tensor(ctx, d->out_tensor);
    Tensor* res = d->res_tensor >= 0 ? get_tensor(ctx, d->res_tensor) : nullptr;
    if (!in) RT_FAIL("op_conv: bad input tensor %d", d->in_tensor);
    if (!d->out_nchw_f32 && !s2d_only && !out) RT_FAIL("op_conv: bad output tensor %d", d->out_tensor);
    if (d->res_tensor >= 0 && !res) RT_FAIL("op_conv: bad residual tensor %d", d->res_tensor);
    if (d->groups < 1 || d->groups > RT_MAX_GROUPS || d->ntaps < 1 || d->ntaps > RT_MAX_TAPS) RT_FAIL("op_conv: groups/ntaps out of range");
    if (d->out_nchw_f32 < 0 || d->out_nchw_f32 > 4) RT_FAIL("op_conv: out_nchw_f32 out of range");
    size_t wbytes = 0, bbytes = 0;
    const f16* w = (const f16*)get_blob(ctx, d->w_blob, &wbytes);
    const float* bias = (const float*)get_blob(ctx, d->bias_blob, &bbytes);
    if (!w || !bias) RT_FAIL("op_conv: bad weight/bias blob");

    Op op;
    ConvKArgs& a = op.conv;
    memset(&a, 0, sizeof(a));
    a.in = in->base; a.wgt = w; a.bias = bias; a.res = res ? res->base : nullptr; a.out = out ? (void*)out->base : nullptr;
    a.HmWm = d->Hm * d->Wm; a.Wm = d->Wm; a.M = in->B * a.HmWm;
    a.in_Hp = in->Hp; a.in_Wp = in->Wp; a.in_C = in->C; a.in_stride = d->in_stride; a.in_P = in->P;
    a.out_scale = d->out_scale;
    if (out) { a.out_Hp = out->Hp; a.out_Wp = out->Wp; a.out_C = out->C; a.out_P = out->P; }
    else { a.out_C = d->cout * d->groups; a.out_H = d->out_H; a.out_W = d->out_W; }
    if (res) { a.res_Hp = res->Hp; a.res_Wp = res->Wp; a.res_C = res->C; a.res_P = res->P; }
    a.cin = d->cin; a.cout = d->cout; a.ntaps = d->ntaps; a.relu = d->relu;
    const int k = d->kernel;
    for (int g = 0; g < d->groups; ++g) {
        for (int t = 0; t < d->ntaps; ++t) {
            const int dy = d->tap_dy[g][t], dx = d->tap_dx[g][t];
            const int ylo = dy, yhi = (d->Hm - 1) * d->in_stride + dy, xlo = dx, xhi = (d->Wm - 1) * d->in_stride + dx;
            const int Hin = d->in_s2d ? 2 * in->H : in->H, Win = d->in_s2d ? 2 * in->W : in->W, Pin = d->in_s2d ? (in->P >= 1 ? 2 : 0) : in->P;
            if (ylo < -Pin || xlo < -Pin || yhi >= Hin + Pin || xhi >= Win + Pin)
                RT_FAIL("op_conv: tap (%d,%d) leaves the padded input (H=%d W=%d pad=%d, Hm=%d Wm=%d stride=%d)", dy, dx, in->H, in->W, in->P, d->Hm, d->Wm, d->in_stride);
            const int dc = d->tap_dc[g][t];
            if (dc && k != RTM3D_CONV_MFMA128 && k != RTM3D_CONV_MFMA256) RT_FAIL("op_conv: per-tap channel offsets need kernel 0 or 2");
            if (!slice_ok(d->in_coff[g] + dc, d->cin, in->C)) RT_FAIL("op_conv: tap %d names channels [%d, %d) outside the %d-channel input tensor", t, d->in_coff[g] + dc, d->in_coff[g] + dc + d->cin, in->C);
            a.g[g].tap_off[t] = (dy * in->Wp + dx) * in->C + dc;
        }
        if (!slice_ok(d->in_coff[g], d->cin, in->C)) RT_FAIL("op_conv: input channel slice out of range");
        const int oyhi = (d->Hm - 1) * d->out_scale + d->out_oy[g], oxhi = (d->Wm - 1) * d->out_scale + d->out_ox[g];
        if (out) {
            if (!slice_ok(d->out_coff[g], d->cout, out->C)) RT_FAIL("op_conv: output channel slice out of range");
            if (oyhi >= out->H || oxhi >= out->W || d->out_oy[g] < 0 || d->out_ox[g] < 0) RT_FAIL("op_conv: output pixel out of range");
            if (out->B != in->B) RT_FAIL("op_conv: batch mismatch");
        } else if (!s2d_only) {
            if (oyhi >= d->out_H || oxhi >= d->out_W || d->out_oy[g] < 0 || d->out_ox[g] < 0) RT_FAIL("op_conv: NCHW output pixel out of range");
            const int c0 = d->out_coff[g], c1 = c0 + d->cout;
            if (c0 < 0 || c1 > d->cout * d->groups) RT_FAIL("op_conv: NCHW output channels [%d,%d) of group %d outside the %d channels of the slot", c0, c1, g, d->cout * d->groups);
            for (int h = 0; h < g; ++h)
                if (d->out_coff[h] < c1 && c0 < d->out_coff[h] + d->cout) RT_FAIL("op_conv: NCHW output channels of groups %d and %d overlap", h, g);
        }
        if (res) {
            if (!slice_ok(d->res_coff[g], d->cout, res->C)) RT_FAIL("op_conv: residual channel slice out of range");
            if (oyhi >= res->H || oxhi >= res->W) RT_FAIL("op_conv: residual pixel out of range");
            if (out && res == out && d->res_coff[g] < d->out_coff[g] + d->cout && d->out_coff[g] < d->res_coff[g] + d->cout)
                RT_FAIL("op_conv: the residual channel slice [%d,%d) overlaps the output slice [%d,%d) of the same tensor", d->res_coff[g], d->res_coff[g] + d->cout, d->out_coff[g], d->out_coff[g] + d->cout);
        }
        a.g[g].in_coff = d->in_coff[g]; a.g[g].out_coff = d->out_coff[g]; a.g[g].res_coff = d->res_coff[g];
        a.g[g].out_oy = d->out_oy[g]; a.g[g].out_ox = d->out_ox[g];
    }
    if (s2d_id >= 0) {
        Tensor* s2 = get_tensor(ctx, s2d_id);
        if (!s2 || (!out && !s2d_only)) RT_FAIL("op_conv: bad space-to-depth tensor %d", s2d_id);
        if ((k != RTM3D_CONV_MFMA128 && k != RTM3D_CONV_C64_HALO) || d->groups != 1 || d->out_scale != 1 || d->out_oy[0] || d->out_ox[0] || (d->Hm & 1) || (d->Wm & 1) || (d->cout % 8))
            RT_FAIL("op_conv: the space-to-depth copy needs kernel 0 or 5, one group, out_scale 1 and an even output height / width");
        if (s2->B != in->B || s2->H * 2 != d->Hm || s2->W * 2 != d->Wm || !slice_ok(d->s2d_coff, 4 * d->cout, s2->C))
            RT_FAIL("op_conv: space-to-depth slice mismatch (half resolution, 4 x cout channels)");
        if (s2 == out || s2 == in || s2 == res) RT_FAIL("op_conv: the space-to-depth copy aliases an operand");
        a.s2d = s2->base; a.s_Hp = s2->Hp; a.s_Wp = s2->Wp; a.s_C = s2->C; a.s_P = s2->P; a.s_coff = d->s2d_coff;
    }
    if (d->in_s2d && k != RTM3D_CONV_C64S2_HALO) RT_FAIL("op_conv: a space-to-depth INPUT is read by kernel 7 only");
    op.groups = d->groups; op.epi_nchw = d->out_nchw_f32 ? 1 : 0; op.out_slot = d->out_nchw_f32 - 1;
    const double M = (double)a.M;
    op.flops = 2.0 * M * d->groups * (double)d->cin * d->ntaps * d->cout;
    op.bytes = 2.0 * M * d->groups * (d->cin + d->cout * (d->out_nchw_f32 ? 2 : 1)) + (res ? 2.0 * M * d->groups * d->cout : 0.0)
               + (s2d_id >= 0 && !s2d_only ? 2.0 * M * d->cout : 0.0);
    int rc;
    switch (k) {
        case RTM3D_CONV_MFMA128: rc = admit_mfma128(ctx, d, wbytes, bbytes, op); break;
        case RTM3D_CONV_MFMA256: rc = admit_mfma256(ctx, d, wbytes, bbytes, op); break;
        case RTM3D_CONV_SMALLC: rc = admit_smallc(ctx, d, wbytes, bbytes, op); break;
        case RTM3D_CONV_C64_HALO: rc = admit_c64_halo(ctx, d, wbytes, bbytes, op); break;
        case RTM3D_CONV_C128_HALO: rc = admit_c128_halo(ctx, d, wbytes, bbytes, op); break;
        case RTM3D_CONV_C64S2_HALO: rc = admit_c64s2_halo(ctx, d, wbytes, bbytes, op); break;
        default: RT_FAIL("op_conv: unknown kernel %d (0 = MFMA 128-px tile, 2 = MFMA 256x256 tile, 3 = register-direct MFMA, 5 / 6 / 7 = halo kernels)", k);
    }
    if (rc) return rc;
    const int stat_slot = d->softmax_stat_slot;
    if (stat_slot >= 0) {
        if (op.kind != OP_CONV_MFMA256) RT_FAIL("op_conv: softmax_stat_slot needs kernel = 2");
        if (stat_slot > 2) RT_FAIL("op_conv: softmax_stat_slot out of range");
        if (conv_mfma256_route(a, d->groups, nullptr) != C256_HALO) RT_FAIL("op_conv: softmax_stat_slot set on a conv that does not take the halo-tile kernel");
        if (d->cout != 256 || out->C != 256) RT_FAIL("op_conv: softmax partials need a 256-channel output tensor");
        for (int g = 0; g < d->groups; ++g) if (d->out_coff[g] != 0) RT_FAIL("op_conv: softmax partials need output channel offset 0");
        const int chunks = d->groups * (d->Hm / 8) * (d->Wm / 32) * 2;
        if (!ctx->stat_buf) {
            RT_HIP(hipMalloc((void**)&ctx->stat_buf, (size_t)3 * in->B * chunks * 256 * 2 * sizeof(float)));
            ctx->extra.push_back(ctx->stat_buf);
            ctx->stat_chunks = chunks; ctx->stat_B = in->B;
        } else if (ctx->stat_chunks != chunks || ctx->stat_B != in->B) {
            RT_FAIL("op_conv: softmax partial producers of one fusion must have equal shapes");
        }
        ctx->stat_tensor[stat_slot] = d->out_tensor;
        op.stat_out = ctx->stat_buf + (size_t)stat_slot * in->B * chunks * 256 * 2;
    }
    ctx->ops.push_back(op);
    return 0;
}

static MxTensor* get_mx8(rtm3d_ctx* ctx, int id) {
    if (id < 0 || id >= (int)ctx->mx8.size()) return nullptr;
    return &ctx->mx8[id];
}

extern "C" int rtm3d_tensor_create_mx8(rtm3d_ctx* ctx, int B, int H, int W, int C, int pad, int* id) {
    if (!ctx || !id) RT_FAIL("tensor_create_mx8: null argument");
    if (B <= 0 || H <= 0 || W <= 0 || C <= 0 || pad < 0 || (C % 32) != 0)
        RT_FAIL("tensor_create_mx8: bad shape B=%d H=%d W=%d C=%d pad=%d (C must be a multiple of 32)", B, H, W, C, pad);
    MxTensor t;
    t.B = B; t.H = H; t.W = W; t.C = C; t.P = pad; t.Hp = H + 2 * pad; t.Wp = W + 2 * pad;
    t.elems = (size_t)B * t.Hp * t.Wp * C;
    if (t.elems >= ((size_t)1 << 32) - 2 * GUARD) RT_FAIL("tensor_create_mx8: %zu bytes exceed the 32-bit offset range of the kernels", t.elems);
    const size_t sbytes = t.elems / 32;
    RT_HIP(hipMalloc((void**)&t.alloc, t.elems + 2 * GUARD));
    RT_HIP(hipMemset(t.alloc, 0, t.elems + 2 * GUARD));
    if (hipMalloc((void**)&t.s_alloc, sbytes + 2 * GUARD) != hipSuccess) { (void)hipFree(t.alloc); RT_FAIL("tensor_create_mx8: out of device memory"); }
    RT_HIP(hipMemset(t.s_alloc, 127, sbytes + 2 * GUARD));
    t.base = t.alloc + GUARD; t.s_base = t.s_alloc + GUARD;
    ctx->mx8.push_back(t);
    *id = (int)ctx->mx8.size() - 1;
    return 0;
}

static float e4m3_to_float(uint8_t b) {
    const int s = b >> 7, e = (b >> 3) & 15, m = b & 7;
    if (e == 15 && m == 7) return NAN;
    const float v = e == 0 ? ldexpf((float)m, -9) : ldexpf((float)(8 + m), e - 10);
    return s ? -v : v;
}

extern "C" int rtm3d_tensor_download_mx8(rtm3d_ctx* ctx, int id, int c0, int C, float* h_nchw) {
    MxTensor* t = ctx ? get_mx8(ctx, id) : nullptr;
    if (!t || !h_nchw || c0 < 0 || C <= 0 || c0 + C > t->C) RT_FAIL("tensor_download_mx8: bad arguments");
    std::vector<uint8_t> d(t->elems), sc(t->elems / 32);
    RT_HIP(hipDeviceSynchronize());
    RT_HIP(hipMemcpy(d.data(), t->base, d.size(), hipMemcpyDeviceToHost));
    RT_HIP(hipMemcpy(sc.data(), t->s_base, sc.size(), hipMemcpyDeviceToHost));
    for (int n = 0; n < t->B; ++n)
        for (int c = 0; c < C; ++c)
            for (int y = 0; y < t->H; ++y)
                for (int x = 0; x < t->W; ++x) {
                    const size_t px = ((size_t)n * t->Hp + y + t->P) * t->Wp + x + t->P;
                    const int cc = c0 + c;
                    h_nchw[(((size_t)n * C + c) * t->H + y) * t->W + x] = ldexpf(e4m3_to_float(d[px * t->C + cc]), (int)sc[px * (t->C / 32) + cc / 32] - 127);
                }
    return 0;
}

static int mx8_raw_copy(rtm3d_ctx* ctx, int id, void* h_data, void* h_scale, bool up) {
    MxTensor* t = ctx ? get_mx8(ctx, id) : nullptr;
    if (!t || !h_data || !h_scale) RT_FAIL("tensor_%sload_mx8_raw: bad arguments", up ? "up" : "down");
    RT_HIP(hipDeviceSynchronize());
    if (up) {
        RT_HIP(hipMemcpy(t->base, h_data, t->elems, hipMemcpyHostToDevice));
        RT_HIP(hipMemcpy(t->s_base, h_scale, t->elems / 32, hipMemcpyHostToDevice));
    } else {
        RT_HIP(hipMemcpy(h_data, t->base, t->elems, hipMemcpyDeviceToHost));
        RT_HIP(hipMemcpy(h_scale, t->s_base, t->elems / 32, hipMemcpyDeviceToHost));
    }
    return 0;
}
extern "C" int rtm3d_tensor_download_mx8_raw(rtm3d_ctx* ctx, int id, void* h_data, void* h_scale) { return mx8_raw_copy(ctx, id, h_data, h_scale, false); }
extern "C" int rtm3d_tensor_upload_mx8_raw(rtm3d_ctx* ctx, int id, const void* h_data, const void* h_scale) {
    return mx8_raw_copy(ctx, id, const_cast<void*>(h_data), const_cast<void*>(h_scale), true);
}

extern "C" int rtm3d_op_quant_mx8(rtm3d_ctx* ctx, int in_tensor, int in_coff, int out_tensor, int out_coff, int channels) {
    Tensor* in = ctx ? get_tensor(ctx, in_tensor) : nullptr;
    MxTensor* o = ctx ? get_mx8(ctx, out_tensor) : nullptr;
    if (!in || !o) RT_FAIL("op_quant_mx8: bad tensors (fp16 input %d, MX8 output %d)", in_tensor, out_tensor);
    if (in->B != o->B || in->H != o->H || in->W != o->W) RT_FAIL("op_quant_mx8: input and output maps differ in shape");
    if (channels <= 0 || channels % 32 || in->C % 8 || !slice_ok(in_coff, channels, in->C))
        RT_FAIL("op_quant_mx8: input slice [%d, %d) of a %d-channel tensor (multiples of 32 channels from a multiple of 8)", in_coff, in_coff + channels, in->C);
    if (out_coff < 0 || out_coff % 32 || out_coff + channels > o->C) RT_FAIL("op_quant_mx8: output slice [%d, %d) (32-channel blocks)", out_coff, out_coff + channels);
    Op op;
    op.kind = OP_QUANT_MX8; op.name = "quant_mx8";
    QuantMx8Args& a = op.qm;
    memset(&a, 0, sizeof(a));
    a.in = in->base; a.out = o->base; a.out_s = o->s_base;
    a.B = in->B; a.H = in->H; a.W = in->W;
    a.in_Hp = in->Hp; a.in_Wp = in->Wp; a.in_C = in->C; a.in_P = in->P; a.in_coff = in_coff;
    a.out_Hp = o->Hp; a.out_Wp = o->Wp; a.out_C = o->C; a.out_P = o->P; a.out_coff = out_coff;
    a.nblk = channels / 32;
    op.flops = 0;
    op.bytes = (double)in->B * in->H * in->W * channels * (2.0 + 1.0 + 1.0 / 32);
    ctx->ops.push_back(op);
    return 0;
}

extern "C" int rtm3d_op_conv_mx8(rtm3d_ctx* ctx, const rtm3d_conv_mx8_desc* d) {
    if (!ctx || !d) RT_FAIL("op_conv_mx8: null argument");
    MxTensor* in = get_mx8(ctx, d->in_tensor);
    if (!in) RT_FAIL("op_conv_mx8: bad MX8 input tensor %d", d->in_tensor);
    if (d->out_fp16 != 0 && d->out_fp16 != 1) RT_FAIL("op_conv_mx8: out_fp16 must be 0 or 1");
    Tensor* of = d->out_fp16 ? get_tensor(ctx, d->out_tensor) : nullptr;
    MxTensor* om = d->out_fp16 ? nullptr : get_mx8(ctx, d->out_tensor);
    if (!of && !om) RT_FAIL("op_conv_mx8: bad %s output tensor %d", d->out_fp16 ? "fp16" : "MX8", d->out_tensor);
    if (om == in) RT_FAIL("op_conv_mx8: the output tensor is the input tensor");
    const int oB = of ? of->B : om->B, oH = of ? of->H : om->H, oW = of ? of->W : om->W, oC = of ? of->C : om->C;
    if (oB != in->B || oH != in->H || oW != in->W) RT_FAIL("op_conv_mx8: input and output maps differ in shape (stride 1, same size)");
    if (d->groups < 1 || d->groups > RT_MAX_GROUPS || d->ntaps < 1 || d->ntaps > RT_MAX_TAPS) RT_FAIL("op_conv_mx8: groups/ntaps out of range");
    if (d->cin <= 0 || d->cin % 64 || d->cout <= 0 || d->cout % 256) RT_FAIL("op_conv_mx8: needs cin %% 64 == 0 and cout %% 256 == 0 (cin=%d cout=%d)", d->cin, d->cout);
    if (in->C % 64) RT_FAIL("op_conv_mx8: the input tensor's channel count %d is not a multiple of 64", in->C);
    for (int t = 0; t < d->ntaps; ++t) {
        const int dy = d->tap_dy[t], dx = d->tap_dx[t];
        if (dy < -in->P || dx < -in->P || in->H - 1 + dy >= in->H + in->P || in->W - 1 + dx >= in->W + in->P)
            RT_FAIL("op_conv_mx8: tap (%d,%d) leaves the padded input (H=%d W=%d pad=%d)", dy, dx, in->H, in->W, in->P);
    }
    for (int g = 0; g < d->groups; ++g) {
        if (d->in_coff[g] < 0 || d->in_coff[g] % 64 || d->in_coff[g] + d->cin > in->C)
            RT_FAIL("op_conv_mx8: input slice [%d, %d) of a %d-channel tensor (offsets multiples of 64)", d->in_coff[g], d->in_coff[g] + d->cin, in->C);
        const int align = of ? 8 : 32;
        if (d->out_coff[g] < 0 || d->out_coff[g] % align || d->out_coff[g] + d->cout > oC)
            RT_FAIL("op_conv_mx8: output slice [%d, %d) of a %d-channel tensor (offsets multiples of %d)", d->out_coff[g], d->out_coff[g] + d->cout, oC, align);
        for (int h = 0; h < g; ++h)
            if (d->out_coff[h] < d->out_coff[g] + d->cout && d->out_coff[g] < d->out_coff[h] + d->cout) RT_FAIL("op_conv_mx8: the output slices of groups %d and %d overlap", h, g);
    }
    const int cpt = d->cin / 64, ksteps = d->ntaps * cpt, NT = d->cout / 256;
    const size_t tiles = (size_t)d->groups * NT * ksteps;
    size_t wb = 0, sb = 0, bb = 0;
    const uint8_t* w = (const uint8_t*)get_blob(ctx, d->w_blob, &wb);
    const uint8_t* ws = (const uint8_t*)get_blob(ctx, d->wscale_blob, &sb);
    const float* bias = (const float*)get_blob(ctx, d->bias_blob, &bb);
    if (!w || !ws || !bias) RT_FAIL("op_conv_mx8: bad weight / scale / bias blob");
    if (wb != tiles * 256 * 64 || sb != tiles * 256 * 2 || bb != (size_t)d->groups * d->cout * sizeof(float))
        RT_FAIL("op_conv_mx8: blob sizes %zu / %zu / %zu, expected %zu / %zu / %zu", wb, sb, bb, tiles * 256 * 64, tiles * 256 * 2, (size_t)d->groups * d->cout * sizeof(float));
    const long long M = (long long)in->B * in->H * in->W;
    if (M >= (1LL << 31)) RT_FAIL("op_conv_mx8: %lld pixels exceed the kernel's 32-bit index", M);
    Op op;
    op.kind = OP_CONV_MX8;
    op.name = d->out_fp16 ? "conv_mx8_to_f16" : "conv_mx8";
    op.groups = d->groups;
    ConvMx8Args& a = op.cm;
    memset(&a, 0, sizeof(a));
    a.in = in->base; a.in_s = in->s_base; a.wgt = w; a.wsc = ws; a.bias = bias;
    a.out = of ? (void*)of->base : (void*)om->base; a.out_s = om ? om->s_base : nullptr;
    a.M = (int)M; a.HmWm = in->H * in->W; a.Wm = in->W;
    a.in_Hp = in->Hp; a.in_Wp = in->Wp; a.in_C = in->C; a.in_P = in->P;
    a.out_Hp = of ? of->Hp : om->Hp; a.out_Wp = of ? of->Wp : om->Wp; a.out_C = oC; a.out_P = of ? of->P : om->P;
    a.cin = d->cin; a.cout = d->cout; a.ntaps = d->ntaps; a.cpt = cpt; a.ksteps = ksteps;
    a.relu = d->relu ? 1 : 0; a.out_fp16 = d->out_fp16;
    a.MT = (int)((M + 255) / 256); a.NT = NT;
    for (int g = 0; g < d->groups; ++g) { a.in_coff[g] = d->in_coff[g]; a.out_coff[g] = d->out_coff[g]; }
    for (int t = 0; t < d->ntaps; ++t) a.tap_pix[t] = d->tap_dy[t] * in->Wp + d->tap_dx[t];
    op.flops = 2.0 * (double)M * d->groups * d->cin * d->ntaps * d->cout;
    op.bytes = (double)M * d->groups * (d->cin * (1.0 + 1.0 / 32) + d->cout * (of ? 2.0 : 1.0 + 1.0 / 32)) + (double)(wb + sb);
    ctx->ops.push_back(op);
    return 0;
}

extern "C" int rtm3d_op_input_nhwc4(rtm3d_ctx* ctx, int out_tensor) {
    Tensor* o = ctx ? get_tensor(ctx, out_tensor) : nullptr;
    if (!o || o->C != 4) RT_FAIL("op_input_nhwc4: output tensor must have 4 channels");
    Op op;
    op.kind = OP_INPUT4; op.name = "nchw_f32_to_nhwc4_f16";
    op.input4 = *o;
    op.flops = 0; op.bytes = (double)o->B * o->H * o->W * (12.0 + 8.0);
    ctx->ops.push_back(op);
    return 0;
}

extern "C" int rtm3d_op_stem_fused(rtm3d_ctx* ctx, int x4_tensor, int out_tensor, int out_coff, int w_base_blob, int b_base_blob,
                                   int w_l0_blob, int b_l0_blob, int w_l1_blob, int b_l1_blob) {
    Tensor* x = ctx ? get_tensor(ctx, x4_tensor) : nullptr;
    Tensor* o = ctx ? get_tensor(ctx, out_tensor) : nullptr;
    if (!x || !o) RT_FAIL("op_stem_fused: bad tensors");
    const bool three = w_l1_blob >= 0;
    const int oc = three ? 32 : 16, sc = three ? 2 : 1;
    if (x->C != 4 || x->P < 4) RT_FAIL("op_stem_fused: the input must be the NHWC4 image tensor with a border >= 4");
    if (o->H * sc != x->H || o->W * sc != x->W || o->B != x->B || !slice_ok(out_coff, oc, o->C)) RT_FAIL("op_stem_fused: output slice mismatch");
    if (x->H % 16 || x->W % 32) RT_FAIL("op_stem_fused: needs H %% 16 == 0 and W %% 32 == 0 (got %dx%d)", x->H, x->W);
    if ((long long)x->H * x->W * 3 * 4 >= (1LL << 31)) RT_FAIL("op_stem_fused: image of %dx%d exceeds the 2 GiB the stem addresses per image", x->H, x->W);
    size_t wb = 0, bb = 0, wl = 0, bl = 0, w1b = 0, b1b = 0;
    const f16* w0 = (const f16*)get_blob(ctx, w_base_blob, &wb);
    const float* b0 = (const float*)get_blob(ctx, b_base_blob, &bb);
    const f16* w1 = (const f16*)get_blob(ctx, w_l0_blob, &wl);
    const float* b1 = (const float*)get_blob(ctx, b_l0_blob, &bl);
    const f16* w2 = three ? (const f16*)get_blob(ctx, w_l1_blob, &w1b) : nullptr;
    const float* b2 = three ? (const float*)get_blob(ctx, b_l1_blob, &b1b) : nullptr;
    if (!w0 || !b0 || !w1 || !b1 || wb != 7 * 64 * 8 * sizeof(f16) || wl != 5 * 64 * 8 * sizeof(f16) || bb != 16 * sizeof(float) || bl != 16 * sizeof(float))
        RT_FAIL("op_stem_fused: weight/bias blob size mismatch");
    if (three && (!w2 || !b2 || w1b != 2 * 5 * 64 * 8 * sizeof(f16) || b1b != 32 * sizeof(float))) RT_FAIL("op_stem_fused: level1 weight/bias blob size mismatch");
    for (auto& prev : ctx->ops)
        if (prev.kind == OP_INPUT4 && prev.input4.base == x->base) prev.input4_unread = true;
    Op op;
    op.kind = OP_STEM_FUSED; op.name = three ? "stem7x7+3x3+3x3s2_fused" : "stem7x7+conv3x3_fused";
    StemFusedArgs& a = op.sf;
    memset(&a, 0, sizeof(a));
    a.x4 = x->base; a.out = o->base; a.w_base = w0; a.w_l0 = w1; a.w_l1 = w2; a.b_base = b0; a.b_l0 = b1; a.b_l1 = b2;
    a.B = x->B; a.H = x->H; a.W = x->W;
    a.x_Hp = x->Hp; a.x_Wp = x->Wp; a.x_P = x->P;
    a.o_Hp = o->Hp; a.o_Wp = o->Wp; a.o_C = o->C; a.o_P = o->P; a.o_coff = out_coff;
    a.tiles_x = x->W / 32; a.tiles_y = x->H / 16;
    const double px = (double)x->B * x->H * x->W;
    op.flops = 2.0 * px * (49.0 * 3 * 16 + 9.0 * 16 * 16 + (three ? 9.0 * 16 * 32 / 4 : 0.0));
    op.bytes = px * (8.0 + (three ? 64.0 / 4 : 32.0));
    ctx->ops.push_back(op);
    return 0;
}

extern "C" int rtm3d_op_conv32s2_fused(rtm3d_ctx* ctx, int in_tensor, int in_coff, int conv_tensor, int conv_coff, int proj_tensor, int proj_coff,
                                       int w_conv_blob, int b_conv_blob, int w_proj_blob, int b_proj_blob) {
    Tensor* x = ctx ? get_tensor(ctx, in_tensor) : nullptr;
    Tensor* oc = ctx ? get_tensor(ctx, conv_tensor) : nullptr;
    Tensor* op_ = ctx ? get_tensor(ctx, proj_tensor) : nullptr;
    if (!x || !oc || !op_) RT_FAIL("op_conv32s2_fused: bad tensors");
    if (x->P < 1 || !slice_ok(in_coff, 32, x->C)) RT_FAIL("op_conv32s2_fused: input slice mismatch (32 channels, border >= 1)");
    if (x->H % 16 || x->W % 64) RT_FAIL("op_conv32s2_fused: needs H %% 16 == 0 and W %% 64 == 0 (got %dx%d)", x->H, x->W);
    for (Tensor* o : {oc, op_})
        if (o->H * 2 != x->H || o->W * 2 != x->W || o->B != x->B) RT_FAIL("op_conv32s2_fused: outputs must have half the input resolution");
    if (!slice_ok(conv_coff, 64, oc->C) || !slice_ok(proj_coff, 64, op_->C)) RT_FAIL("op_conv32s2_fused: output slice mismatch");
    if (oc == op_ && conv_coff < proj_coff + 64 && proj_coff < conv_coff + 64)
        RT_FAIL("op_conv32s2_fused: the conv slice [%d,%d) overlaps the project slice [%d,%d) of the same tensor", conv_coff, conv_coff + 64, proj_coff, proj_coff + 64);
    size_t wc = 0, bc = 0, wp = 0, bp = 0;
    const f16* w0 = (const f16*)get_blob(ctx, w_conv_blob, &wc);
    const float* b0 = (const float*)get_blob(ctx, b_conv_blob, &bc);
    const f16* w1 = (const f16*)get_blob(ctx, w_proj_blob, &wp);
    const float* b1 = (const float*)get_blob(ctx, b_proj_blob, &bp);
    if (!w0 || !b0 || !w1 || !b1 || wc != 9 * 4 * 64 * 8 * sizeof(f16) || wp != 4 * 64 * 8 * sizeof(f16) || bc != 64 * sizeof(float) || bp != 64 * sizeof(float))
        RT_FAIL("op_conv32s2_fused: weight/bias blob size mismatch");
    Op op;
    if (claim_ticket(ctx, op, "op_conv32s2_fused")) return 1;
    op.kind = OP_CONV32S2_FUSED; op.name = "pool+proj1x1+conv3x3s2_fused";
    Conv32S2Args& a = op.c32;
    memset(&a, 0, sizeof(a));
    a.in = x->base; a.out_conv = oc->base; a.out_proj = op_->base; a.w_conv = w0; a.w_proj = w1; a.b_conv = b0; a.b_proj = b1;
    a.B = x->B; a.Ho = oc->H; a.Wo = oc->W;
    a.in_Hp = x->Hp; a.in_Wp = x->Wp; a.in_C = x->C; a.in_P = x->P; a.in_coff = in_coff;
    a.oc_Hp = oc->Hp; a.oc_Wp = oc->Wp; a.oc_C = oc->C; a.oc_P = oc->P; a.oc_coff = conv_coff;
    a.op_Hp = op_->Hp; a.op_Wp = op_->Wp; a.op_C = op_->C; a.op_P = op_->P; a.op_coff = proj_coff;
    const double opx = (double)x->B * oc->H * oc->W;
    op.flops = 2.0 * opx * (9.0 * 32 * 64 + 32.0 * 64);
    op.bytes = opx * (4 * 64.0 + 2 * 128.0);
    ctx->ops.push_back(op);
    return 0;
}

extern "C" int rtm3d_op_conv64_root(rtm3d_ctx* ctx, int in_tensor, int in_coff, int res_tensor, int res_coff, int conv_relu,
                                    int w_conv_blob, int b_conv_blob, int w_root_blob, int b_root_blob,
                                    int out_tensor, int out_coff, int root_relu, int pool_tensor, int pool_coff,
                                    int s2d_tensor, int s2d_coff) {
    Tensor* in = ctx ? get_tensor(ctx, in_tensor) : nullptr;
    Tensor* res = ctx ? get_tensor(ctx, res_tensor) : nullptr;
    Tensor* out = ctx && out_tensor >= 0 ? get_tensor(ctx, out_tensor) : nullptr;
    Tensor* pool = ctx && pool_tensor >= 0 ? get_tensor(ctx, pool_tensor) : nullptr;
    Tensor* s2d = ctx && s2d_tensor >= 0 ? get_tensor(ctx, s2d_tensor) : nullptr;
    if (!in || !res || (out_tensor >= 0 && !out) || (pool_tensor >= 0 && !pool) || (s2d_tensor >= 0 && !s2d)) RT_FAIL("op_conv64_root: bad tensors");
    if (!out && !s2d) RT_FAIL("op_conv64_root: out_tensor < 0 (no ordinary copy of the root output) needs a space-to-depth copy");
    if (s2d) {
        if (s2d->H * 2 != in->H || s2d->W * 2 != in->W || s2d->B != in->B || !slice_ok(s2d_coff, 256, s2d->C))
            RT_FAIL("op_conv64_root: space-to-depth output slice mismatch (half resolution, 4 x 64 channels)");
        if (s2d == out || s2d == res || s2d == in) RT_FAIL("op_conv64_root: the space-to-depth copy aliases an operand");
    }
    if (in->P < 1 || !slice_ok(in_coff, 64, in->C)) RT_FAIL("op_conv64_root: input slice mismatch (64 channels, border >= 1)");
    if (in->H % 8 || in->W % 32) RT_FAIL("op_conv64_root: needs H %% 8 == 0 and W %% 32 == 0 (got %dx%d)", in->H, in->W);
    for (Tensor* t : {res, out})
        if (t && (t->H != in->H || t->W != in->W || t->B != in->B)) RT_FAIL("op_conv64_root: residual / output shape mismatch");
    if (!slice_ok(res_coff, 64, res->C) || (out && !slice_ok(out_coff, 64, out->C))) RT_FAIL("op_conv64_root: residual / output slice mismatch");
    if (out && res == out && res_coff < out_coff + 64 && out_coff < res_coff + 64) RT_FAIL("op_conv64_root: the root output overlaps x1 (another workgroup may still read it)");
    if (out && in == out && in_coff < out_coff + 64 && out_coff < in_coff + 64) RT_FAIL("op_conv64_root: the root output overlaps the conv input");
    if (pool) {
        if (pool->H * 2 != in->H || pool->W * 2 != in->W || pool->B != in->B || !slice_ok(pool_coff, 64, pool->C))
            RT_FAIL("op_conv64_root: pooled output slice mismatch (half resolution, 64 channels)");
        if (s2d && pool == s2d && pool_coff < s2d_coff + 256 && s2d_coff < pool_coff + 64)
            RT_FAIL("op_conv64_root: the pooled slice [%d,%d) overlaps the space-to-depth slice [%d,%d) of the same tensor", pool_coff, pool_coff + 64, s2d_coff, s2d_coff + 256);
        if (pool == in || pool == res || (out && pool == out)) RT_FAIL("op_conv64_root: the pooled output aliases an operand");
    }
    size_t wc = 0, bc = 0, wr = 0, br = 0;
    const f16* w0 = (const f16*)get_blob(ctx, w_conv_blob, &wc);
    const float* b0 = (const float*)get_blob(ctx, b_conv_blob, &bc);
    const f16* w1 = (const f16*)get_blob(ctx, w_root_blob, &wr);
    const float* b1 = (const float*)get_blob(ctx, b_root_blob, &br);
    if (!w0 || !b0 || !w1 || !b1 || wc != (size_t)9 * 64 * 64 * sizeof(f16) || bc != 64 * sizeof(float) || wr != (size_t)64 * 128 * sizeof(f16) || br != 64 * sizeof(float))
        RT_FAIL("op_conv64_root: weight/bias blob size mismatch");
    Op op;
    if (claim_ticket(ctx, op, "op_conv64_root")) return 1;
    ConvKArgs& a = op.conv;
    memset(&a, 0, sizeof(a));
    a.in = in->base; a.wgt = w0; a.bias = b0; a.res = res->base; a.out = nullptr;
    a.HmWm = in->H * in->W; a.Wm = in->W; a.M = in->B * a.HmWm;
    a.in_Hp = in->Hp; a.in_Wp = in->Wp; a.in_C = in->C; a.in_stride = 1; a.in_P = in->P; a.out_scale = 1;
    a.res_Hp = res->Hp; a.res_Wp = res->Wp; a.res_C = res->C; a.res_P = res->P;
    a.cin = 64; a.cout = 64; a.ntaps = 9; a.relu = conv_relu ? 1 : 0; a.cpt = 1; a.ksteps = 9; a.NT = 1;
    for (int t = 0; t < 9; ++t) a.g[0].tap_off[t] = ((t / 3 - 1) * in->Wp + (t % 3 - 1)) * in->C;
    a.g[0].in_coff = in_coff; a.g[0].res_coff = res_coff;
    RootKArgs& r = op.root;
    memset(&r, 0, sizeof(r));
    r.w = w1; r.bias = b1;
    if (out) { r.out = out->base; r.o_Hp = out->Hp; r.o_Wp = out->Wp; r.o_C = out->C; r.o_P = out->P; r.o_coff = out_coff; }
    r.relu = root_relu ? 1 : 0;
    if (pool) { r.pool = pool->base; r.p_Hp = pool->Hp; r.p_Wp = pool->Wp; r.p_C = pool->C; r.p_P = pool->P; r.p_coff = pool_coff; }
    if (s2d) { r.s2d = s2d->base; r.s_Hp = s2d->Hp; r.s_Wp = s2d->Wp; r.s_C = s2d->C; r.s_P = s2d->P; r.s_coff = s2d_coff; }
    op.kind = OP_CONV64_ROOT; op.groups = 1; op.bn_tile = 64; op.epi_nchw = 0; op.out_slot = -1;
    op.name = pool ? "conv3x3_c64+root1x1+pool_fused" : "conv3x3_c64+root1x1_fused";
    if (s2d) op.name += "+s2d";
    const double M = (double)a.M;
    op.flops = 2.0 * M * (9.0 * 64 * 64 + 128.0 * 64);
    op.bytes = 2.0 * M * (64.0 * 2 + (out ? 64.0 : 0.0) + (pool ? 16.0 : 0.0) + (s2d ? 64.0 : 0.0));
    ctx->ops.push_back(op);
    return 0;
}

extern "C" int rtm3d_op_patch_mask(rtm3d_ctx* ctx, int tensor, int yx_blob, int img_H, int img_W, int origin) {
    Tensor* t = ctx ? get_tensor(ctx, tensor) : nullptr;
    if (!t) RT_FAIL("op_patch_mask: bad tensor");
    if (t->P != 0 || t->H != t->W || (t->C % 8) || img_H < 1 || img_W < 1 || origin < 0 || origin >= t->H) RT_FAIL("op_patch_mask: the patch tensor must be square, borderless, with a multiple of 8 channels");
    size_t bytes = 0;
    const int32_t* yx = (const int32_t*)get_blob(ctx, yx_blob, &bytes);
    if (!yx || bytes < (size_t)t->B * 2 * sizeof(int32_t)) RT_FAIL("op_patch_mask: the (y, x) blob needs 2 int32 per slot");
    Op op;
    op.kind = OP_PATCH_MASK; op.name = "patch_mask";
    op.pm.base = t->base; op.pm.yx = yx; op.pm.n_slots = t->B; op.pm.S = t->H; op.pm.C = t->C;
    op.pm.img_H = img_H; op.pm.img_W = img_W; op.pm.origin = origin;
    op.flops = 0; op.bytes = 0;
    ctx->ops.push_back(op);
    return 0;
}

extern "C" int rtm3d_op_headout(rtm3d_ctx* ctx, int in_tensor, int w_blob, int bias_blob, int nheads, const int* cout4) {
    Tensor* in = ctx ? get_tensor(ctx, in_tensor) : nullptr;
    if (!in || !cout4) RT_FAIL("op_headout: bad arguments");
    if (nheads < 1 || nheads > 4) RT_FAIL("op_headout: nheads must be in [1,4]");
    if (in->C != 256 * nheads || in->P < 1) RT_FAIL("op_headout: input must be the nheads x 256 channel head tensor with a border >= 1");
    size_t wb = 0, bb = 0;
    const f16* w = (const f16*)get_blob(ctx, w_blob, &wb);
    const float* b = (const float*)get_blob(ctx, bias_blob, &bb);
    if (!w || !b || wb != (size_t)nheads * 9 * 8 * 64 * 8 * sizeof(f16) || bb != (size_t)nheads * 16 * sizeof(float)) RT_FAIL("op_headout: weight/bias blob size mismatch");
    Op op;
    op.kind = OP_HEADOUT; op.name = "conv3x3_headout_halo";
    HeadOutArgs& a = op.ho;
    memset(&a, 0, sizeof(a));
    a.in = in->base; a.wgt = w; a.bias = b;
    int csum = 0;
    for (int i = 0; i < nheads; ++i) { if (cout4[i] < 1 || cout4[i] > 16) RT_FAIL("op_headout: cout must be in [1,16]"); a.cout[i] = cout4[i]; csum += cout4[i]; }
    a.nheads = nheads;
    a.B = in->B; a.H = in->H; a.W = in->W;
    a.in_Hp = in->Hp; a.in_Wp = in->Wp; a.in_C = in->C; a.in_P = in->P;
    a.tile_rows = (long long)in->B * ((in->H + 15) / 16) * ((in->W + 31) / 32) * nheads >= 4LL * ctx->n_cus ? 16 : 8;
    a.tiles_x = (in->W + 31) / 32; a.tiles_y = (in->H + a.tile_rows - 1) / a.tile_rows;
    op.flops = 2.0 * in->B * in->H * in->W * 9.0 * 256.0 * csum;
    op.bytes = (double)in->B * in->H * in->W * (256.0 * nheads * 2 + csum * 4.0);
    ctx->ops.push_back(op);
    return 0;
}

extern "C" int rtm3d_op_maxpool(rtm3d_ctx* ctx, int in_tensor, int in_coff, int out_tensor, int out_coff,
                                int channels, int ksize, int stride, int pad) {
    Tensor* in = ctx ? get_tensor(ctx, in_tensor) : nullptr;
    Tensor* out = ctx ? get_tensor(ctx, out_tensor) : nullptr;
    if (!in || !out) RT_FAIL("op_maxpool: bad tensors");
    if (channels % 8 || in_coff % 8 || out_coff % 8 || in_coff + channels > in->C || out_coff + channels > out->C) RT_FAIL("op_maxpool: bad channel slice");
    if (pad > in->P) RT_FAIL("op_maxpool: input border %d narrower than pool padding %d", in->P, pad);
    if ((out->H - 1) * stride - pad + ksize - 1 >= in->H + in->P || (out->W - 1) * stride - pad + ksize - 1 >= in->W + in->P) RT_FAIL("op_maxpool: window leaves the padded input");
    Op op;
    op.kind = OP_MAXPOOL; op.name = "maxpool";
    PoolKArgs& a = op.pool;
    a.in = in->base; a.out = out->base; a.B = in->B; a.Ho = out->H; a.Wo = out->W; a.C8 = channels / 8;
    a.in_Hp = in->Hp; a.in_Wp = in->Wp; a.in_C = in->C; a.in_P = in->P; a.in_coff = in_coff;
    a.out_Hp = out->Hp; a.out_Wp = out->Wp; a.out_C = out->C; a.out_P = out->P; a.out_coff = out_coff;
    a.ksize = ksize; a.stride = stride; a.pad = pad;
    op.flops = 0;
    op.bytes = 2.0 * in->B * channels * ((double)in->H * in->W + (double)out->H * out->W);
    ctx->ops.push_back(op);
    return 0;
}

extern "C" int rtm3d_op_maxpool_s2d(rtm3d_ctx* ctx, int in_tensor, int in_coff, int out_tensor, int out_coff, int channels) {
    Tensor* in = ctx ? get_tensor(ctx, in_tensor) : nullptr;
    Tensor* out = ctx ? get_tensor(ctx, out_tensor) : nullptr;
    if (!in || !out) RT_FAIL("op_maxpool_s2d: bad tensors");
    if (channels % 8 || !slice_ok(in_coff, 4 * channels, in->C) || !slice_ok(out_coff, channels, out->C)) RT_FAIL("op_maxpool_s2d: bad channel slices (input: 4 x channels)");
    if (in->H != out->H || in->W != out->W || in->B != out->B) RT_FAIL("op_maxpool_s2d: the space-to-depth copy and the pooled map have one resolution");
    if (in == out && in_coff < out_coff + channels && out_coff < in_coff + 4 * channels) RT_FAIL("op_maxpool_s2d: output overlaps the input slices");
    Op op;
    op.kind = OP_MAXPOOL; op.name = "maxpool_s2d";
    PoolKArgs& a = op.pool;
    a.in = in->base; a.out = out->base; a.B = in->B; a.Ho = out->H; a.Wo = out->W; a.C8 = channels / 8;
    a.in_Hp = in->Hp; a.in_Wp = in->Wp; a.in_C = in->C; a.in_P = in->P; a.in_coff = in_coff;
    a.out_Hp = out->Hp; a.out_Wp = out->Wp; a.out_C = out->C; a.out_P = out->P; a.out_coff = out_coff;
    a.ksize = 0; a.stride = 0; a.pad = 0;
    op.flops = 0;
    op.bytes = 2.0 * in->B * channels * 5.0 * (double)out->H * out->W;
    ctx->ops.push_back(op);
    return 0;
}

extern "C" int rtm3d_op_softmax_fuse(rtm3d_ctx* ctx, int z_in, int z_out, int n_u, const int* u_tensors) {
    Tensor* zi = ctx ? get_tensor(ctx, z_in) : nullptr;
    Tensor* zo = ctx ? get_tensor(ctx, z_out) : nullptr;
    if (!zi || !zo || n_u < 1 || n_u > 3 || !u_tensors) RT_FAIL("op_softmax_fuse: bad arguments");
    if (zi->C != 256 || zo->C != 256 || zi->H != zo->H || zi->W != zo->W || zi->B != zo->B) RT_FAIL("op_softmax_fuse: z tensors must be 256-channel with equal shape");
    Op op;
    op.kind = OP_SOFTMAX; op.name = "softmax_fuse";
    SoftmaxKArgs& a = op.sm;
    memset(&a, 0, sizeof(a));
    a.z_in = zi->base; a.z_out = zo->base; a.n_u = n_u;
    a.B = zi->B; a.H = zi->H; a.W = zi->W; a.C = 256;
    a.z_Hp = zo->Hp; a.z_Wp = zo->Wp; a.z_C = zo->C; a.z_P = zo->P;
    a.zi_Hp = zi->Hp; a.zi_Wp = zi->Wp; a.zi_C = zi->C; a.zi_P = zi->P;
    for (int i = 0; i < n_u; ++i) {
        Tensor* u = get_tensor(ctx, u_tensors[i]);
        if (!u || u->C != 256 || u->H != zi->H || u->W != zi->W || u->B != zi->B) RT_FAIL("op_softmax_fuse: u tensor %d mismatch", i);
        a.u[i] = u->base; a.u_Hp[i] = u->Hp; a.u_Wp[i] = u->Wp; a.u_C[i] = u->C; a.u_P[i] = u->P;
    }
    const bool small = (long long)a.B * ((a.H + 1) / 2) < 2LL * ctx->n_cus;
    a.rows_per_chunk = small ? 1 : 2;
    a.chunks = (a.H + a.rows_per_chunk - 1) / a.rows_per_chunk;
    a.apply_rows = 1; a.xsplit = 1;
    while (a.xsplit < 4 && a.W / (a.xsplit * 2) >= 64) a.xsplit *= 2;
    while ((long long)a.B * a.H * a.xsplit < 2LL * ctx->n_cus && a.xsplit < 8 && a.W / (a.xsplit * 2) >= 32) a.xsplit *= 2;
    a.seg_w = ((a.W + a.xsplit - 1) / a.xsplit + 7) / 8 * 8;
    a.apply_chunks = a.H * a.xsplit;
    bool emitted = ctx->stat_buf != nullptr && ctx->stat_B == a.B;
    for (int i = 0; i < n_u && emitted; ++i) emitted = ctx->stat_tensor[i] == u_tensors[i];
    for (int i = 0; i < 3; ++i) if ((i < n_u) != (ctx->stat_tensor[i] >= 0) && ctx->stat_buf) emitted = false;
    if (ctx->stat_buf && !emitted) RT_FAIL("op_softmax_fuse: the recorded softmax_stat_slot producers do not match this fusion's operands");
    if (emitted) {
        a.partial = ctx->stat_buf;
        a.partial_chunks = ctx->stat_chunks;
        ctx->stat_buf = nullptr;
        ctx->stat_tensor[0] = ctx->stat_tensor[1] = ctx->stat_tensor[2] = -1;
    } else {
        void* part = nullptr;
        RT_HIP(hipMalloc(&part, (size_t)n_u * a.B * a.chunks * a.C * 2 * sizeof(float)));
        ctx->extra.push_back(part);
        a.partial = (float*)part;
        a.partial_chunks = 0;
    }
    void* st = nullptr;
    RT_HIP(hipMalloc(&st, (size_t)n_u * a.B * a.C * 2 * sizeof(float)));
    ctx->extra.push_back(st);
    a.stats = (float*)st;
    op.flops = 0;
    op.bytes = 2.0 * a.B * a.H * a.W * 256.0 * ((emitted ? 1.0 : 2.0) * n_u + 2.0);
    ctx->ops.push_back(op);
    return 0;
}

static int launch_op(rtm3d_ctx* ctx, Op& op, hipStream_t s, const float* d_in, float* const d_out[4]) {
    hipError_t e = hipSuccess;
    unsigned int* const ctr256 = ctx->tile_ctr;
    switch (op.kind) {
        case OP_CONV_MFMA: {
            ConvKArgs a = op.conv;
            if (op.epi_nchw) a.out = d_out[op.out_slot];
            e = a.deep ? launch_conv_mfma_deep(a, op.bn_tile, op.groups, split_ctrs(ctx), s)
                       : launch_conv_mfma(a, op.bn_tile, op.groups, op.epi_nchw, s);
            break;
        }
        case OP_CONV_MFMA256: e = launch_conv_mfma256(op.conv, op.groups, ctr256, op.stat_out, s); break;
        case OP_CONV64_HALO: e = launch_conv64_halo(op.conv, ctx->n_cus, ticket_ctr(ctx, op), s); break;
        case OP_CONV64S2_HALO: e = launch_conv64s2_halo(op.conv, ctx->n_cus, ticket_ctr(ctx, op), s); break;
        case OP_CONV64_ROOT: e = launch_conv64_root(op.conv, op.root, ctx->n_cus, ticket_ctr(ctx, op), s); break;
        case OP_CONV128_HALO: e = launch_conv128_halo(op.conv, ctx->n_cus, ticket_ctr(ctx, op), s); break;
        case OP_STEM_FUSED: {
            StemFusedArgs a = op.sf;
            a.x_nchw = d_in;
            e = launch_stem_fused(a, s);
            break;
        }
        case OP_CONV32S2_FUSED: e = launch_conv32s2_fused(op.c32, ctx->n_cus, ticket_ctr(ctx, op), s); break;
        case OP_CONV_SMALLC: e = launch_conv_smallc(op.conv, s); break;
        case OP_INPUT4: if (!d_in || op.input4_unread) break;
            e = launch_nchw_to_nhwc4(d_in, op.input4.base, op.input4.B, op.input4.H, op.input4.W, op.input4.Hp, op.input4.Wp, op.input4.P, s); break;
        case OP_HEADOUT: {
            HeadOutArgs a = op.ho;
            for (int i = 0; i < 4; ++i) a.out[i] = d_out[i];
            e = launch_conv_headout(a, s);
            break;
        }
        case OP_MAXPOOL: e = launch_maxpool(op.pool, s); break;
        case OP_SOFTMAX: e = launch_softmax_fuse(op.sm, s); break;
        case OP_PATCH_MASK: e = launch_patch_mask(op.pm, s); break;
        case OP_QUANT_MX8: e = launch_quant_mx8(op.qm, s); break;
        case OP_CONV_MX8: e = launch_conv_mx8(op.cm, op.groups, s); break;
    }
    if (e != hipSuccess) { rt_set_error("launch of op '%s' failed: %s", op.name.c_str(), hipGetErrorString(e)); return 1; }
    return 0;
}

__global__ void zero_words_kernel(unsigned int* __restrict__ p, int n) {
    const int i = blockIdx.x * 256 + threadIdx.x;
    if (i < n) p[i] = 0u;
}
static hipError_t zero_counters(rtm3d_ctx* ctx, hipStream_t s) {
    if (!ctx->tile_ctr) return hipSuccess;
    hipLaunchKernelGGL(zero_words_kernel, dim3(((int)TILE_CTR_WORDS + 255) / 256), dim3(256), 0, s, ctx->tile_ctr, (int)TILE_CTR_WORDS);
    return hipGetLastError();
}

static int replay_eager(rtm3d_ctx* ctx, hipStream_t s, const float* d_in, float* const d_out_logits[4], bool probes) {
    RT_HIP(zero_counters(ctx, s));
    if (ctx->test_memset_in_replay && ctx->tile_ctr) RT_HIP(hipMemsetAsync(ctx->tile_ctr, 0, sizeof(unsigned int), s));
    const int n = (int)ctx->ops.size();
    for (int i = 0; i < n; ++i) {
        Op& op = ctx->ops[i];
        for (int m = 0; m < ctx->n_marks; ++m)
            if (ctx->mark_op[m] == i) RT_HIP(hipEventRecord(ctx->mark_ev[m], s));
        const bool probe = probes && (i == ctx->probe_op);
        const int slot = ctx->probe_count % PROBE_RING;
        if (probe) RT_HIP(hipEventRecord(ctx->probe_ev[2 * slot], s));
        if (launch_op(ctx, op, s, d_in, d_out_logits)) return 1;
        if (probe) { RT_HIP(hipEventRecord(ctx->probe_ev[2 * slot + 1], s)); ctx->probe_count++; }
    }
    if (ctx->n_marks) RT_HIP(hipEventRecord(ctx->mark_ev[ctx->n_marks], s));
    return 0;
}

static const size_t GRAPH_CACHE = 8;

static int graph_non_kernel_nodes(hipGraph_t graph) {
    size_t n = 0;
    if (hipGraphGetNodes(graph, nullptr, &n) != hipSuccess) return -1;
    std::vector<hipGraphNode_t> nodes(n);
    if (n && hipGraphGetNodes(graph, nodes.data(), &n) != hipSuccess) return -1;
    int bad = 0;
    for (size_t i = 0; i < n; ++i) {
        hipGraphNodeType ty;
        if (hipGraphNodeGetType(nodes[i], &ty) != hipSuccess) return -1;
        if (ty != hipGraphNodeTypeKernel) ++bad;
    }
    return bad;
}

static int forward_on_stream(rtm3d_ctx* ctx, hipStream_t s, const float* d_in, float* const d_out_logits[4]);

static int replay_begin(rtm3d_ctx* ctx, hipStream_t s) {
    if (ctx->has_last && ctx->last_stream != s) RT_HIP(hipStreamWaitEvent(s, ctx->done_ev, 0));
    return 0;
}
static int replay_end(rtm3d_ctx* ctx, hipStream_t s) {
    if (!ctx->done_ev) RT_HIP(hipEventCreateWithFlags(&ctx->done_ev, hipEventDisableTiming));
    RT_HIP(hipEventRecord(ctx->done_ev, s));
    ctx->last_stream = s; ctx->has_last = true;
    return 0;
}

extern "C" int rtm3d_forward(rtm3d_ctx* ctx, void* stream, const float* d_in, float* const d_out_logits[4]) {
    if (!ctx || !d_out_logits) RT_FAIL("forward: null argument");
    if (!d_out_logits[0]) RT_FAIL("forward: null logits buffer 0");
    if (ctx->ops.empty()) RT_FAIL("forward: empty plan");
    hipStream_t s = (hipStream_t)stream;
    if (replay_begin(ctx, s)) return 1;
    const int rc = forward_on_stream(ctx, s, d_in, d_out_logits);
    if (replay_end(ctx, s)) return 1;
    return rc;
}

static int forward_on_stream(rtm3d_ctx* ctx, hipStream_t s, const float* d_in, float* const d_out_logits[4]) {
    if (!ctx->graph_mode || ctx->probe_op >= 0) return replay_eager(ctx, s, d_in, d_out_logits, true);
    const void* key[5] = {d_in, d_out_logits[0], d_out_logits[1], d_out_logits[2], d_out_logits[3]};
    ctx->graph_clock++;
    for (auto& ge : ctx->graphs)
        if (!memcmp(ge.key, key, sizeof(key))) { ge.last_use = ctx->graph_clock; ctx->graph_hits++; RT_HIP(hipGraphLaunch(ge.exec, s)); return 0; }
    if (++ctx->graph_captures > 32 && ctx->graph_hits < ctx->graph_captures) { ctx->graph_mode = 0; return replay_eager(ctx, s, d_in, d_out_logits, true); }
    if (!ctx->capture_stream) RT_HIP(hipStreamCreateWithFlags(&ctx->capture_stream, hipStreamNonBlocking));
    RT_HIP(hipStreamBeginCapture(ctx->capture_stream, hipStreamCaptureModeThreadLocal));
    const int rc = replay_eager(ctx, ctx->capture_stream, d_in, d_out_logits, false);
    hipGraph_t graph = nullptr;
    const hipError_t ec = hipStreamEndCapture(ctx->capture_stream, &graph);
    if (rc) { if (graph) (void)hipGraphDestroy(graph); return 1; }
    if (ec != hipSuccess) { rt_set_error("forward: graph capture failed: %s", hipGetErrorString(ec)); return 1; }
    {
        int bad = graph_non_kernel_nodes(graph);
        if (bad != 0) {
            (void)hipGraphDestroy(graph);
            ctx->graph_mode = 0;
            ctx->graph_refused++;
            rt_set_error("forward: the captured plan holds %d non-kernel graph node(s) (memset / memcpy nodes are not allowed in a replay graph); graph mode is off for this context", bad);
            return replay_eager(ctx, s, d_in, d_out_logits, true);
        }
    }
    rtm3d_ctx::GraphEntry ge;
    memcpy(ge.key, key, sizeof(key));
    ge.graph = graph;
    const hipError_t ei = hipGraphInstantiate(&ge.exec, graph, nullptr, nullptr, 0);
    if (ei != hipSuccess) { (void)hipGraphDestroy(graph); rt_set_error("forward: hipGraphInstantiate failed: %s", hipGetErrorString(ei)); return 1; }
    ge.last_use = ctx->graph_clock;
    if (ctx->graphs.size() >= GRAPH_CACHE) {
        size_t lru = 0;
        for (size_t i = 1; i < ctx->graphs.size(); ++i) if (ctx->graphs[i].last_use < ctx->graphs[lru].last_use) lru = i;
        (void)hipGraphExecDestroy(ctx->graphs[lru].exec); (void)hipGraphDestroy(ctx->graphs[lru].graph);
        ctx->graphs[lru] = ge;
    } else {
        ctx->graphs.push_back(ge);
    }
    RT_HIP(hipGraphLaunch(ge.exec, s));
    return 0;
}

extern "C" int rtm3d_input_tensor(rtm3d_ctx* ctx, void** d_base, int* B, int* H, int* W, int* border) {
    if (!ctx || !d_base || !B || !H || !W || !border) RT_FAIL("input_tensor: null argument");
    for (auto& op : ctx->ops)
        if (op.kind == OP_INPUT4) {
            *d_base = op.input4.base; *B = op.input4.B; *H = op.input4.H; *W = op.input4.W; *border = op.input4.P;
            return 0;
        }
    RT_FAIL("input_tensor: the plan has no NHWC4 input tensor");
}

extern "C" int rtm3d_ctx_set_graph(rtm3d_ctx* ctx, int enable) {
    if (!ctx) RT_FAIL("ctx_set_graph: null context");
    ctx->graph_mode = enable ? 1 : 0;
    return 0;
}

extern "C" int rtm3d_ctx_graph_stats(rtm3d_ctx* ctx, int* captures, int* hits, int* enabled) {
    if (!ctx) RT_FAIL("ctx_graph_stats: null context");
    if (captures) *captures = (int)ctx->graph_captures;
    if (hits) *hits = (int)ctx->graph_hits;
    if (enabled) *enabled = ctx->graph_mode;
    return 0;
}

extern "C" int rtm3d_ctx_debug_memset_in_replay(rtm3d_ctx* ctx, int enable) {
    if (!ctx) RT_FAIL("ctx_debug_memset_in_replay: null context");
    if (ensure_tile_ctr(ctx)) return 1;
    ctx->test_memset_in_replay = enable ? 1 : 0;
    return 0;
}

extern "C" int rtm3d_ctx_debug_read_words(rtm3d_ctx* ctx, int offset, int n, unsigned int* h_out) {
    if (!ctx || !h_out || offset < 0 || n < 1 || (size_t)offset + (size_t)n > DEBUG_WORDS) RT_FAIL("ctx_debug_read_words: bad arguments");
    if (ensure_tile_ctr(ctx)) return 1;
    RT_HIP(hipDeviceSynchronize());
    RT_HIP(hipMemcpy(h_out, ctx->tile_ctr + DEBUG_WORD0 + offset, (size_t)n * sizeof(unsigned int), hipMemcpyDeviceToHost));
    return 0;
}

extern "C" int rtm3d_probe_set(rtm3d_ctx* ctx, int op_index) {
    if (!ctx || op_index >= (int)ctx->ops.size()) RT_FAIL("probe_set: bad op index");
    if (ctx->probe_ev.empty() && op_index >= 0) {
        ctx->probe_ev.resize(2 * PROBE_RING);
        for (auto& e : ctx->probe_ev) RT_HIP(hipEventCreate(&e));
    }
    ctx->probe_op = op_index;
    ctx->probe_count = 0;
    return 0;
}

extern "C" int rtm3d_probe_read(rtm3d_ctx* ctx, double* avg_ms, int* count) {
    if (!ctx || !avg_ms || !count) RT_FAIL("probe_read: null argument");
    const int n = ctx->probe_count < PROBE_RING ? ctx->probe_count : PROBE_RING;
    double sum = 0.0;
    for (int i = 0; i < n; ++i) {
        float ms = 0.f;
        RT_HIP(hipEventSynchronize(ctx->probe_ev[2 * i + 1]));
        RT_HIP(hipEventElapsedTime(&ms, ctx->probe_ev[2 * i], ctx->probe_ev[2 * i + 1]));
        sum += ms;
    }
    *avg_ms = n ? sum / n : 0.0;
    *count = n;
    return 0;
}

extern "C" int rtm3d_forward_timed(rtm3d_ctx* ctx, void* stream, const float* d_in, float* const d_out_logits[4],
                                   float* h_ms, int cap, int* n_ops) {
    if (!ctx || !d_out_logits) RT_FAIL("forward_timed: null argument");
    const int n = (int)ctx->ops.size();
    if (n_ops) *n_ops = n;
    if (!h_ms) return 0;
    if (cap < n) RT_FAIL("forward_timed: capacity %d < %d ops", cap, n);
    if (!d_out_logits[0]) RT_FAIL("forward_timed: null logits buffer 0");
    std::vector<hipEvent_t> ev(n + 1, nullptr);
    hipStream_t s = (hipStream_t)stream;
    int rc = 0;
    hipError_t e = hipSuccess;
    for (auto& v : ev) if ((e = hipEventCreate(&v)) != hipSuccess) { rc = 1; break; }
    if (!rc && replay_begin(ctx, s)) rc = 2;
    if (!rc) {
        if ((e = zero_counters(ctx, s)) != hipSuccess) rc = 1;
        if (!rc && (e = hipEventRecord(ev[0], s)) != hipSuccess) rc = 1;
        for (int i = 0; i < n && !rc; ++i) {
            if (launch_op(ctx, ctx->ops[i], s, d_in, d_out_logits)) { rc = 2; break; }
            if ((e = hipEventRecord(ev[i + 1], s)) != hipSuccess) rc = 1;
        }
        if (replay_end(ctx, s) && !rc) rc = 2;
        if (!rc && (e = hipEventSynchronize(ev[n])) != hipSuccess) rc = 1;
        for (int i = 0; i < n && !rc; ++i) if ((e = hipEventElapsedTime(&h_ms[i], ev[i], ev[i + 1])) != hipSuccess) rc = 1;
    }
    for (auto& v : ev) if (v) (void)hipEventDestroy(v);
    if (rc == 1) rt_set_error("forward_timed: %s", hipGetErrorString(e));
    return rc ? 1 : 0;
}

extern "C" int rtm3d_forward_marks(rtm3d_ctx* ctx, void* stream, const float* d_in, float* const d_out_logits[4],
                                   int n_marks, const int* mark_ops, float* h_ms) {
    if (!ctx || !d_out_logits || !d_out_logits[0] || !mark_ops || !h_ms || n_marks < 1 || n_marks > 8) RT_FAIL("forward_marks: bad arguments");
    for (int i = 0; i < n_marks; ++i)
        if (mark_ops[i] < 0 || mark_ops[i] >= (int)ctx->ops.size() || (i && mark_ops[i] <= mark_ops[i - 1]))
            RT_FAIL("forward_marks: mark %d (op %d) must be an ascending op index", i, mark_ops[i]);
    hipStream_t s = (hipStream_t)stream;
    int rc = 0;
    hipError_t e = hipSuccess;
    for (int i = 0; i <= n_marks && !rc; ++i) { ctx->mark_ev[i] = nullptr; if ((e = hipEventCreate(&ctx->mark_ev[i])) != hipSuccess) rc = 1; }
    if (!rc) {
        for (int i = 0; i < n_marks; ++i) ctx->mark_op[i] = mark_ops[i];
        ctx->n_marks = n_marks;
        if (replay_begin(ctx, s)) rc = 2;
        if (!rc && replay_eager(ctx, s, d_in, d_out_logits, true)) rc = 2;
        ctx->n_marks = 0;
        if (replay_end(ctx, s) && !rc) rc = 2;
        if (!rc && (e = hipEventSynchronize(ctx->mark_ev[n_marks])) != hipSuccess) rc = 1;
        for (int i = 0; i < n_marks && !rc; ++i) if ((e = hipEventElapsedTime(&h_ms[i], ctx->mark_ev[i], ctx->mark_ev[i + 1])) != hipSuccess) rc = 1;
    }
    ctx->n_marks = 0;
    for (int i = 0; i <= n_marks; ++i) if (ctx->mark_ev[i]) { (void)hipEventDestroy(ctx->mark_ev[i]); ctx->mark_ev[i] = nullptr; }
    if (rc == 1) rt_set_error("forward_marks: %s", hipGetErrorString(e));
    return rc ? 1 : 0;
}

extern "C" int rtm3d_op_info(rtm3d_ctx* ctx, int i, double* flops, double* bytes, const char** name) {
    if (!ctx || i < 0 || i >= (int)ctx->ops.size()) RT_FAIL("op_info: index out of range");
    if (flops) *flops = ctx->ops[i].flops;
    if (bytes) *bytes = ctx->ops[i].bytes;
    if (name) *name = ctx->ops[i].name.c_str();
    return 0;
}

extern "C" int rtm3d_stream_create_cumask(int device, int n_cus, void** stream) {
    if (!stream || n_cus < 1) RT_FAIL("stream_create_cumask: bad arguments");
    RT_HIP(hipSetDevice(device));
    hipDeviceProp_t prop;
    RT_HIP(hipGetDeviceProperties(&prop, device));
    const int total = prop.multiProcessorCount;
    if (n_cus > total) n_cus = total;
    const int words = (total + 31) / 32;
    std::vector<uint32_t> mask(words, 0u);
    for (int i = 0; i < n_cus; ++i) mask[i >> 5] |= 1u << (i & 31);
    hipStream_t s = nullptr;
    RT_HIP(hipExtStreamCreateWithCUMask(&s, (uint32_t)words, mask.data()));
    *stream = (void*)s;
    return 0;
}

extern "C" int rtm3d_stream_destroy(void* stream) {
    if (stream) RT_HIP(hipStreamDestroy((hipStream_t)stream));
    return 0;
}
```

Measured before the change: 2687.

## Fold softmax apply into the producing 256-channel persistent conv epilogue

The conv that produces the softmax input is deferred until after the softmax reduce/combine stats kernels, then launched with an epilogue that applies the softmax-weighted sum of the u tensors directly to its accumulators and writes z_out. This drops the separate apply kernel and the round trip of writing and re-reading z_in. Runtime gains read/write dependency tracking so it can check that the reorder is legal and undo the fold when a later op reads z_in. The cost is heavier epilogue register use and extra u-tensor loads inside the conv kernel.

```diff
diff --git a/rtm3d_amd/csrc/common.h b/rtm3d_amd/csrc/common.h
--- a/rtm3d_amd/csrc/common.h
+++ b/rtm3d_amd/csrc/common.h
@@ -93,6 +93,20 @@
     int chunks, rows_per_chunk;
     int apply_chunks, apply_rows, xsplit, seg_w;
     int partial_chunks;
+    int stats_only;
+};
+
+__device__ __forceinline__ float softmax_apply_elem(float acc, float f, float M, float invS) {
+    return __builtin_fmaf(f, __expf(f - M) * invS, acc);
+}
+
+struct ApplyFoldArgs {
+    const f16* u[3];
+    f16* z_out;
+    const float* stats;
+    int n_u, B;
+    uint32_t u_img[3], u_row[3];
+    uint32_t z_img, z_row;
 };
 
 __device__ __forceinline__ int xcd_contiguous_index(int b, int n) {
@@ -197,6 +211,7 @@
 hipError_t launch_conv_mfma(const ConvKArgs& a, int bn_tile, int groups, int epi_nchw, hipStream_t s);
 hipError_t launch_conv_mfma_deep(const ConvKArgs& a, int bn_tile, int groups, unsigned int* tile_ctr, hipStream_t s);
 hipError_t launch_conv_mfma256(const ConvKArgs& a, int groups, unsigned int* tile_ctr, float* stat_out, hipStream_t s);
+hipError_t launch_conv_mfma256_apply(const ConvKArgs& a, int groups, const ApplyFoldArgs& f, unsigned int* tile_ctr, hipStream_t s);
 enum Conv256Route { C256_ONE_TILE, C256_PERSISTENT, C256_HALO, C256_LATTICE };
 Conv256Route conv_mfma256_route(const ConvKArgs& a, int groups, HaloTaps* ht);
 void conv_mfma256_permute_weights(const f16* src, f16* dst, size_t n_ktiles);
diff --git a/rtm3d_amd/csrc/conv_mfma256.hip b/rtm3d_amd/csrc/conv_mfma256.hip
--- a/rtm3d_amd/csrc/conv_mfma256.hip
+++ b/rtm3d_amd/csrc/conv_mfma256.hip
@@ -321,8 +321,21 @@
         sp ^= 1;                                                                            \
     }
 
+struct C256PersistentKernargs { ConvKArgs a; int groups, nbias; unsigned int* tile_ctr; int one_list; ApplyFoldArgs af; };
+#define CONST_AS __attribute__((address_space(4)))
+#ifndef C256_APPLY_RUNS
+#define C256_APPLY_RUNS 1
+#endif
+#ifdef C256_T_APPLY_PLAIN
+#define C256_APPLY_LOAD(p) (*(p))
+#else
+#define C256_APPLY_LOAD(p) __builtin_nontemporal_load(p)
+#endif
 template <int RES, int XNT>
-__global__ __launch_bounds__(512) void conv_mfma256_persistent_kernel(const ConvKArgs a, const int groups, const int nbias, unsigned int* tile_ctr, const int one_list) {
+__global__ __launch_bounds__(512) void conv_mfma256_persistent_kernel(const ConvKArgs a, const int groups, const int nbias, unsigned int* tile_ctr, const int one_list,
+                                                                      const ApplyFoldArgs af) {
+    constexpr int NU = RES >= 2 ? RES - 1 : 0, NUA = NU ? NU : 1;
+    constexpr bool ADD_RES = RES == 1;
     __shared__ __attribute__((aligned(16))) f16 lds[2 * BUF_ELEMS + HALF_ELEMS];
     __shared__ __attribute__((aligned(16))) float lds_bias[CONV256_MAX_BIAS + 4];
 #ifdef C256_STAMPS
@@ -508,7 +521,94 @@
         if (wave < 4) __builtin_amdgcn_s_barrier();
         TSTAMP(1)
 
-        {
+        if constexpr (NU > 0) {
+            uintptr_t kp = (uintptr_t)__builtin_amdgcn_kernarg_segment_ptr() + offsetof(C256PersistentKernargs, af);
+            asm volatile("" : "+s"(kp));
+            const CONST_AS ApplyFoldArgs& F = *(const CONST_AS ApplyFoldArgs*)kp;
+            uint32_t tid16 = wvoff;
+            asm volatile("" : "+v"(tid16));
+            const int frow_e = (int)(tid16 >> 4) & 15, fk_e = (int)(tid16 >> 8) & 3;
+            const uint32_t cb2 = (uint32_t)(wc * 64 + frow_e * 4) * 2u;
+            const int g_oy = a.g[gi_c].out_oy, g_ox = a.g[gi_c].out_ox;
+            auto load_stats = [&](int ui, int n, f32x4 (&st)[2]) {
+                const GLB_AS f32x4* sp = (const GLB_AS f32x4*)((uintptr_t)F.stats + ((size_t)(ui * F.B + n) * 2048u + cb2 * 4u));
+                st[0] = sp[0]; st[1] = sp[1];
+            };
+            auto fused = [&](int i, int p, int e, const f16x4 (&uv)[NUA], const f32x4 (&st)[NUA][2]) -> f16x4 {
+                const f32x4 vv = {acc[i][0][0][p][e], acc[i][0][1][p][e], acc[i][1][0][p][e], acc[i][1][1][p][e]};
+                f16x4 h = {(f16)vv[0], (f16)vv[1], (f16)vv[2], (f16)vv[3]};
+                h = __builtin_elementwise_max(h, lo4);
+                f16x4 o;
+#pragma unroll
+                for (int k = 0; k < 4; ++k) {
+                    float z = (float)h[k];
+#pragma unroll
+                    for (int ui = 0; ui < NU; ++ui) z = softmax_apply_elem(z, (float)uv[ui][k], st[ui][k >> 1][(k & 1) * 2], st[ui][k >> 1][(k & 1) * 2 + 1]);
+                    asm volatile("" : "+v"(z));
+                    o[k] = (f16)z;
+                }
+                return o;
+            };
+            const int mfirst = mt_c * 256, mlast = mfirst + 255 < a.M ? mfirst + 255 : a.M - 1;
+            const int n_tile = div_small_q(mfirst, a.HmWm, rcp_hw);
+            if (mlast < (n_tile + 1) * a.HmWm) {
+                f32x4 st[NUA][2];
+                uintptr_t ub[NUA];
+#pragma unroll
+                for (int ui = 0; ui < NU; ++ui) { load_stats(ui, n_tile, st[ui]); ub[ui] = (uintptr_t)F.u[ui] + (size_t)n_tile * F.u_img[ui]; }
+                const uintptr_t zb = (uintptr_t)F.z_out + (size_t)n_tile * F.z_img;
+#pragma unroll
+                for (int i = 0; i < 2; ++i)
+#pragma unroll
+                    for (int ph = 0; ph < 4 / C256_APPLY_RUNS; ++ph) {
+                        uint32_t zo[C256_APPLY_RUNS][4];
+                        f16x4 uv[C256_APPLY_RUNS][4][NUA];
+#pragma unroll
+                        for (int pq = 0; pq < C256_APPLY_RUNS; ++pq) {
+                            const int m0 = mt_c * 256 + i * 128 + wp * 64 + (ph * C256_APPLY_RUNS + pq) * 16 + fk_e * 4;
+                            const int m = m0 < a.M ? m0 : a.M - 1;
+                            int n = n_tile;
+                            const int rem = m - n * a.HmWm;
+                            int y = div_small_q(rem, a.Wm, rcp_w), x = rem - y * a.Wm;
+#pragma unroll
+                            for (int e = 0; e < 4; ++e) {
+                                if (e) c256_next_pixel(n, y, x, m0 + e < a.M, a.Wm, Hm);
+                                const uint32_t oy = (uint32_t)(y * a.out_scale + g_oy), xc = (uint32_t)(x * a.out_scale + g_ox) * 512u + cb2;
+                                zo[pq][e] = oy * F.z_row + xc;
+#pragma unroll
+                                for (int ui = 0; ui < NU; ++ui)
+                                    uv[pq][e][ui] = C256_APPLY_LOAD((const GLB_AS f16x4*)(ub[ui] + (oy * F.u_row[ui] + xc)));
+                            }
+                        }
+#pragma unroll
+                        for (int pq = 0; pq < C256_APPLY_RUNS; ++pq)
+#pragma unroll
+                            for (int e = 0; e < 4; ++e)
+                                *(GLB_AS f16x4*)(zb + zo[pq][e]) = fused(i, ph * C256_APPLY_RUNS + pq, e, uv[pq][e], st);
+                    }
+            } else {
+#pragma unroll
+                for (int i = 0; i < 2; ++i)
+#pragma unroll
+                    for (int p = 0; p < 4; ++p)
+#pragma unroll
+                        for (int e = 0; e < 4; ++e) {
+                            const int m0 = mt_c * 256 + i * 128 + wp * 64 + p * 16 + fk_e * 4 + e;
+                            const int m = m0 < a.M ? m0 : a.M - 1;
+                            const int n = div_small_q(m, a.HmWm, rcp_hw), rem = m - n * a.HmWm;
+                            const int y = div_small_q(rem, a.Wm, rcp_w), x = rem - y * a.Wm;
+                            const uint32_t oy = (uint32_t)(y * a.out_scale + g_oy), xc = (uint32_t)(x * a.out_scale + g_ox) * 512u + cb2;
+                            f32x4 st[NUA][2];
+                            f16x4 uv[NUA];
+#pragma unroll
+                            for (int ui = 0; ui < NU; ++ui) {
+                                load_stats(ui, n, st[ui]);
+                                uv[ui] = C256_APPLY_LOAD((const GLB_AS f16x4*)((uintptr_t)F.u[ui] + ((uint32_t)n * F.u_img[ui] + oy * F.u_row[ui] + xc)));
+                            }
+                            *(GLB_AS f16x4*)((uintptr_t)F.z_out + ((uint32_t)n * F.z_img + oy * F.z_row + xc)) = fused(i, p, e, uv, st);
+                        }
+            }
+        } else {
             const ConvGroupArgs& g = a.g[gi_c];
             const int cbase = nt_c * 256 + wc * 64 + frow * 4;
 #pragma unroll
@@ -527,7 +627,7 @@
                         if (e) c256_next_pixel(n, y, x, m0 + e < a.M, a.Wm, Hm);
                         const int oy = y * a.out_scale + g.out_oy, ox = x * a.out_scale + g.out_ox;
                         opix[p][e] = ((size_t)(n * a.out_Hp + oy + a.out_P) * a.out_Wp + ox + a.out_P) * a.out_C + g.out_coff + cbase;
-                        if (RES) rv[p][e] = *(const f16x4*)(a.res + ((size_t)(n * a.res_Hp + oy + a.res_P) * a.res_Wp + ox + a.res_P) * a.res_C + g.res_coff + cbase);
+                        if (ADD_RES) rv[p][e] = *(const f16x4*)(a.res + ((size_t)(n * a.res_Hp + oy + a.res_P) * a.res_Wp + ox + a.res_P) * a.res_C + g.res_coff + cbase);
                     }
                 }
 #pragma unroll
@@ -535,7 +635,7 @@
 #pragma unroll
                     for (int e = 0; e < 4; ++e) {
                         f32x4 vv = {acc[i][0][0][p][e], acc[i][0][1][p][e], acc[i][1][0][p][e], acc[i][1][1][p][e]};
-                        if (RES) {
+                        if (ADD_RES) {
                             const f16x4 r = rv[p][e];
                             vv[0] += (float)r[0]; vv[1] += (float)r[1]; vv[2] += (float)r[2]; vv[3] += (float)r[3];
                         }
@@ -605,6 +705,31 @@
     if (nbias <= 1024 && conv_mfma256_lattice_dilation(a, groups) != 0) return C256_LATTICE;
 #endif
     return C256_PERSISTENT;
+}
+
+template <int RES, int XNT>
+static hipError_t launch_persistent(const ConvKArgs& a, int groups, int nbias, unsigned int* tile_ctr, const ApplyFoldArgs& af, hipStream_t s) {
+    const int per_xcd = device_cu_count() / 8;
+    const int one_list = (long long)a.MT * a.NT * groups <= device_cu_count() ? 1 : 0;
+    hipLaunchKernelGGL((conv_mfma256_persistent_kernel<RES, XNT>), dim3(per_xcd * 8, 1, 1), dim3(512, 1, 1), 0, s, a, groups, nbias, tile_ctr, one_list, af);
+    return hipGetLastError();
+}
+
+hipError_t launch_conv_mfma256_apply(const ConvKArgs& a, int groups, const ApplyFoldArgs& f, unsigned int* tile_ctr, hipStream_t s) {
+    if (f.n_u < 1 || f.n_u > 3 || !f.z_out || !f.stats || !tile_ctr || groups < 1 || groups > RT_MAX_GROUPS || a.res || a.NT != 1 || a.cout != 256 ||
+        conv_mfma256_route(a, groups, nullptr) != C256_PERSISTENT)
+        return hipErrorInvalidValue;
+    for (int g = 0; g < groups; ++g) if (a.g[g].out_coff != 0) return hipErrorInvalidValue;
+    const int nbias = conv256_nbias(a, groups);
+    const bool x_once = a.ntaps == 1 && a.in_stride == 1;
+    switch (f.n_u * 2 + (x_once ? 1 : 0)) {
+        case 2: return launch_persistent<2, 0>(a, groups, nbias, tile_ctr, f, s);
+        case 3: return launch_persistent<2, 1>(a, groups, nbias, tile_ctr, f, s);
+        case 4: return launch_persistent<3, 0>(a, groups, nbias, tile_ctr, f, s);
+        case 5: return launch_persistent<3, 1>(a, groups, nbias, tile_ctr, f, s);
+        case 6: return launch_persistent<4, 0>(a, groups, nbias, tile_ctr, f, s);
+        default: return launch_persistent<4, 1>(a, groups, nbias, tile_ctr, f, s);
+    }
 }
 
 hipError_t launch_conv_mfma256(const ConvKArgs& a, int groups, unsigned int* tile_ctr, float* stat_out, hipStream_t s) {
@@ -617,14 +742,11 @@
     if (route == C256_HALO) return launch_conv_mfma256_halo(a, ht, groups, nbias, device_cu_count(), tile_ctr, stat_out, s);
     if (route == C256_LATTICE) return launch_conv_mfma256_lattice(a, groups, nbias, device_cu_count(), tile_ctr, s);
     if (route == C256_PERSISTENT) {
-        const int per_xcd = device_cu_count() / 8;
-        const int one_list = (long long)a.MT * a.NT * groups <= device_cu_count() ? 1 : 0;
-        dim3 grid(per_xcd * 8, 1, 1);
         const bool x_once = !a.res && a.ntaps == 1 && a.NT == 1 && a.in_stride == 1;
-        if (a.res) hipLaunchKernelGGL((conv_mfma256_persistent_kernel<1, 0>), grid, block, 0, s, a, groups, nbias, tile_ctr, one_list);
-        else if (x_once) hipLaunchKernelGGL((conv_mfma256_persistent_kernel<0, 1>), grid, block, 0, s, a, groups, nbias, tile_ctr, one_list);
-        else hipLaunchKernelGGL((conv_mfma256_persistent_kernel<0, 0>), grid, block, 0, s, a, groups, nbias, tile_ctr, one_list);
-        return hipGetLastError();
+        const ApplyFoldArgs none = {};
+        if (a.res) return launch_persistent<1, 0>(a, groups, nbias, tile_ctr, none, s);
+        if (x_once) return launch_persistent<0, 1>(a, groups, nbias, tile_ctr, none, s);
+        return launch_persistent<0, 0>(a, groups, nbias, tile_ctr, none, s);
     }
     const int mt8 = (a.MT + 7) / 8 * 8;
     dim3 grid(mt8 * a.NT, groups, 1);
diff --git a/rtm3d_amd/csrc/pool_softmax.hip b/rtm3d_amd/csrc/pool_softmax.hip
--- a/rtm3d_amd/csrc/pool_softmax.hip
+++ b/rtm3d_amd/csrc/pool_softmax.hip
@@ -156,7 +156,7 @@
 #pragma unroll
                     for (int ui = 0; ui < NU; ++ui) {
                         const float f = (float)v[k][ui][e];
-                        acc += f * (__expf(f - M[ui][e]) * invS[ui][e]);
+                        acc = softmax_apply_elem(acc, f, M[ui][e], invS[ui][e]);
                     }
                     o[e] = (f16)acc;
                 }
@@ -170,6 +170,7 @@
     if (a.C != 256 || a.n_u < 1 || a.n_u > 3 || a.xsplit < 1 || a.seg_w < 1 || a.apply_rows < 1) return hipErrorInvalidValue;
     if (a.partial_chunks <= 0) hipLaunchKernelGGL(softmax_reduce_kernel, dim3(a.chunks, a.B, a.n_u), dim3(256), 0, s, a);
     hipLaunchKernelGGL(softmax_combine_kernel, dim3(a.B, a.n_u, a.C / 64), dim3(1024), 0, s, a);
+    if (a.stats_only) return hipGetLastError();
     if (a.n_u == 3) hipLaunchKernelGGL(softmax_apply_kernel<3>, dim3(a.apply_chunks, a.B, 1), dim3(256), 0, s, a);
     else if (a.n_u == 2) hipLaunchKernelGGL(softmax_apply_kernel<2>, dim3(a.apply_chunks, a.B, 1), dim3(256), 0, s, a);
     else hipLaunchKernelGGL(softmax_apply_kernel<1>, dim3(a.apply_chunks, a.B, 1), dim3(256), 0, s, a);
diff --git a/rtm3d_amd/csrc/runtime.hip b/rtm3d_amd/csrc/runtime.hip
--- a/rtm3d_amd/csrc/runtime.hip
+++ b/rtm3d_amd/csrc/runtime.hip
@@ -1,6 +1,7 @@
 #include <math.h>
 #include <stdarg.h>
 #include <stdio.h>
+#include <stdlib.h>
 #include <string.h>
 #include <string>
 #include <vector>
@@ -43,6 +44,11 @@
     ConvKArgs conv; int groups, bn_tile, epi_nchw, out_slot;
     int ticket_slot = -1;
     float* stat_out = nullptr;
+    std::vector<int> reads, writes;
+    bool deferred = false;
+    int fold_conv = -1;
+    ApplyFoldArgs af;
+    double own_flops = 0, own_bytes = 0;
     Tensor input4;
     bool input4_unread = false;
     PoolKArgs pool;
@@ -245,6 +251,24 @@
     if (id < 0 || id >= (int)ctx->blobs.size()) return nullptr;
     if (bytes) *bytes = ctx->blob_bytes[id];
     return ctx->blobs[id];
+}
+
+static void undo_apply_fold(rtm3d_ctx* ctx, int si) {
+    Op& sm = ctx->ops[si];
+    if (sm.fold_conv < 0) return;
+    Op& cv = ctx->ops[sm.fold_conv];
+    cv.deferred = false; cv.flops = cv.own_flops; cv.bytes = cv.own_bytes;
+    sm.fold_conv = -1; sm.sm.stats_only = 0; sm.flops = sm.own_flops; sm.bytes = sm.own_bytes;
+}
+
+static void record_op(rtm3d_ctx* ctx, Op& op, std::initializer_list<int> reads, std::initializer_list<int> writes) {
+    for (int id : reads) if (id >= 0) op.reads.push_back(id);
+    for (int id : writes) if (id >= 0) op.writes.push_back(id);
+    for (size_t i = 0; i < ctx->ops.size(); ++i)
+        if (ctx->ops[i].fold_conv >= 0)
+            for (int id : op.reads)
+                if (id == ctx->ops[i].reads[0]) undo_apply_fold(ctx, (int)i);
+    ctx->ops.push_back(op);
 }
 
 static int admit_mfma128(rtm3d_ctx* ctx, const rtm3d_conv_desc* d, size_t wbytes, size_t bbytes, Op& op) {
@@ -510,7 +534,7 @@
         ctx->stat_tensor[stat_slot] = d->out_tensor;
         op.stat_out = ctx->stat_buf + (size_t)stat_slot * in->B * chunks * 256 * 2;
     }
-    ctx->ops.push_back(op);
+    record_op(ctx, op, {d->in_tensor, d->res_tensor}, {out ? d->out_tensor : -1, s2d_id});
     return 0;
 }
 
@@ -600,7 +624,7 @@
     a.nblk = channels / 32;
     op.flops = 0;
     op.bytes = (double)in->B * in->H * in->W * channels * (2.0 + 1.0 + 1.0 / 32);
-    ctx->ops.push_back(op);
+    record_op(ctx, op, {in_tensor}, {});
     return 0;
 }
 
@@ -661,7 +685,7 @@
     for (int t = 0; t < d->ntaps; ++t) a.tap_pix[t] = d->tap_dy[t] * in->Wp + d->tap_dx[t];
     op.flops = 2.0 * (double)M * d->groups * d->cin * d->ntaps * d->cout;
     op.bytes = (double)M * d->groups * (d->cin * (1.0 + 1.0 / 32) + d->cout * (of ? 2.0 : 1.0 + 1.0 / 32)) + (double)(wb + sb);
-    ctx->ops.push_back(op);
+    record_op(ctx, op, {}, {of ? d->out_tensor : -1});
     return 0;
 }
 
@@ -672,7 +696,7 @@
     op.kind = OP_INPUT4; op.name = "nchw_f32_to_nhwc4_f16";
     op.input4 = *o;
     op.flops = 0; op.bytes = (double)o->B * o->H * o->W * (12.0 + 8.0);
-    ctx->ops.push_back(op);
+    record_op(ctx, op, {}, {out_tensor});
     return 0;
 }
 
@@ -711,7 +735,7 @@
     const double px = (double)x->B * x->H * x->W;
     op.flops = 2.0 * px * (49.0 * 3 * 16 + 9.0 * 16 * 16 + (three ? 9.0 * 16 * 32 / 4 : 0.0));
     op.bytes = px * (8.0 + (three ? 64.0 / 4 : 32.0));
-    ctx->ops.push_back(op);
+    record_op(ctx, op, {x4_tensor}, {out_tensor});
     return 0;
 }
 
@@ -748,7 +772,7 @@
     const double opx = (double)x->B * oc->H * oc->W;
     op.flops = 2.0 * opx * (9.0 * 32 * 64 + 32.0 * 64);
     op.bytes = opx * (4 * 64.0 + 2 * 128.0);
-    ctx->ops.push_back(op);
+    record_op(ctx, op, {in_tensor}, {conv_tensor, proj_tensor});
     return 0;
 }
 
@@ -813,7 +837,7 @@
     const double M = (double)a.M;
     op.flops = 2.0 * M * (9.0 * 64 * 64 + 128.0 * 64);
     op.bytes = 2.0 * M * (64.0 * 2 + (out ? 64.0 : 0.0) + (pool ? 16.0 : 0.0) + (s2d ? 64.0 : 0.0));
-    ctx->ops.push_back(op);
+    record_op(ctx, op, {in_tensor, res_tensor}, {out_tensor, pool_tensor, s2d_tensor});
     return 0;
 }
 
@@ -829,7 +853,7 @@
     op.pm.base = t->base; op.pm.yx = yx; op.pm.n_slots = t->B; op.pm.S = t->H; op.pm.C = t->C;
     op.pm.img_H = img_H; op.pm.img_W = img_W; op.pm.origin = origin;
     op.flops = 0; op.bytes = 0;
-    ctx->ops.push_back(op);
+    record_op(ctx, op, {tensor}, {tensor});
     return 0;
 }
 
@@ -856,7 +880,7 @@
     a.tiles_x = (in->W + 31) / 32; a.tiles_y = (in->H + a.tile_rows - 1) / a.tile_rows;
     op.flops = 2.0 * in->B * in->H * in->W * 9.0 * 256.0 * csum;
     op.bytes = (double)in->B * in->H * in->W * (256.0 * nheads * 2 + csum * 4.0);
-    ctx->ops.push_back(op);
+    record_op(ctx, op, {in_tensor}, {});
     return 0;
 }
 
@@ -877,7 +901,7 @@
     a.ksize = ksize; a.stride = stride; a.pad = pad;
     op.flops = 0;
     op.bytes = 2.0 * in->B * channels * ((double)in->H * in->W + (double)out->H * out->W);
-    ctx->ops.push_back(op);
+    record_op(ctx, op, {in_tensor}, {out_tensor});
     return 0;
 }
 
@@ -897,8 +921,51 @@
     a.ksize = 0; a.stride = 0; a.pad = 0;
     op.flops = 0;
     op.bytes = 2.0 * in->B * channels * 5.0 * (double)out->H * out->W;
-    ctx->ops.push_back(op);
-    return 0;
+    record_op(ctx, op, {in_tensor}, {out_tensor});
+    return 0;
+}
+
+static int apply_fold_producer(rtm3d_ctx* ctx, int z_in, int z_out, int n_u, const int* u_tensors) {
+    const char* off = getenv("RTM3D_NO_APPLY_FOLD");
+    if (off && off[0] && strcmp(off, "0") != 0) return -1;
+    if (z_out == z_in) return -1;
+    Tensor* zi = get_tensor(ctx, z_in);
+    Tensor* zo = get_tensor(ctx, z_out);
+    if ((zo->elems + 2 * GUARD) * sizeof(f16) >= ((size_t)1 << 32)) return -1;
+    for (int i = 0; i < n_u; ++i) {
+        if (u_tensors[i] == z_out || u_tensors[i] == z_in) return -1;
+        if ((get_tensor(ctx, u_tensors[i])->elems + 2 * GUARD) * sizeof(f16) >= ((size_t)1 << 32)) return -1;
+    }
+    const int n = (int)ctx->ops.size();
+    int ci = -1;
+    for (int i = n - 1; i >= 0 && ci < 0; --i)
+        for (int id : ctx->ops[i].writes) if (id == z_in) ci = i;
+    if (ci < 0) return -1;
+    const Op& cv = ctx->ops[ci];
+    const ConvKArgs& c = cv.conv;
+    if (cv.kind != OP_CONV_MFMA256 || cv.deferred || cv.epi_nchw || cv.stat_out) return -1;
+    if (conv_mfma256_route(c, cv.groups, nullptr) != C256_PERSISTENT) return -1;
+    if (c.res || c.s2d || c.NT != 1 || c.cout != 256 || c.out_C != 256) return -1;
+    const int sc = c.out_scale;
+    if (sc < 1 || sc > 2 || cv.groups != sc * sc || c.out != (void*)zi->base || cv.writes.size() != 1) return -1;
+    if (c.Wm * sc != zi->W || c.HmWm * sc * sc != zi->H * zi->W || c.M != zi->B * c.HmWm) return -1;
+    unsigned phases = 0;
+    for (int g = 0; g < cv.groups; ++g) {
+        const ConvGroupArgs& cg = c.g[g];
+        if (cg.out_coff != 0 || cg.out_oy < 0 || cg.out_oy >= sc || cg.out_ox < 0 || cg.out_ox >= sc) return -1;
+        phases |= 1u << (cg.out_oy * sc + cg.out_ox);
+    }
+    if (phases != (1u << (sc * sc)) - 1) return -1;
+    for (int id : cv.reads) if (id == z_out) return -1;
+    for (int i = ci + 1; i < n; ++i) {
+        const Op& o = ctx->ops[i];
+        for (int id : o.reads) if (id == z_in || id == z_out) return -1;
+        for (int id : o.writes) {
+            if (id == z_out) return -1;
+            for (int rd : cv.reads) if (id == rd) return -1;
+        }
+    }
+    return ci;
 }
 
 extern "C" int rtm3d_op_softmax_fuse(rtm3d_ctx* ctx, int z_in, int z_out, int n_u, const int* u_tensors) {
@@ -949,7 +1016,31 @@
     a.stats = (float*)st;
     op.flops = 0;
     op.bytes = 2.0 * a.B * a.H * a.W * 256.0 * ((emitted ? 1.0 : 2.0) * n_u + 2.0);
-    ctx->ops.push_back(op);
+    op.own_flops = op.flops; op.own_bytes = op.bytes;
+    const int ci = apply_fold_producer(ctx, z_in, z_out, n_u, u_tensors);
+    if (ci >= 0) {
+        Op& cv = ctx->ops[ci];
+        ApplyFoldArgs& f = op.af;
+        memset(&f, 0, sizeof(f));
+        auto origin = [](Tensor* t) { return t->base + ((size_t)t->P * t->Wp + t->P) * t->C; };
+        for (int i = 0; i < n_u; ++i) {
+            Tensor* u = get_tensor(ctx, u_tensors[i]);
+            f.u[i] = origin(u); f.u_img[i] = (uint32_t)((size_t)u->Hp * u->Wp * 512); f.u_row[i] = (uint32_t)((size_t)u->Wp * 512);
+        }
+        f.z_out = origin(zo); f.z_img = (uint32_t)((size_t)zo->Hp * zo->Wp * 512); f.z_row = (uint32_t)((size_t)zo->Wp * 512);
+        f.stats = a.stats; f.n_u = n_u; f.B = a.B;
+        a.stats_only = 1;
+        op.fold_conv = ci;
+        cv.own_flops = cv.flops; cv.own_bytes = cv.bytes;
+        cv.deferred = true;
+        op.flops += cv.flops;
+        op.bytes += cv.bytes - 2.0 * (2.0 * a.B * a.H * a.W * 256.0);
+        cv.flops = 0; cv.bytes = 0;
+    }
+    std::initializer_list<int> none = {};
+    op.reads.push_back(z_in);
+    for (int i = 0; i < n_u; ++i) op.reads.push_back(u_tensors[i]);
+    record_op(ctx, op, none, {z_out});
     return 0;
 }
 
@@ -964,7 +1055,9 @@
                        : launch_conv_mfma(a, op.bn_tile, op.groups, op.epi_nchw, s);
             break;
         }
-        case OP_CONV_MFMA256: e = launch_conv_mfma256(op.conv, op.groups, ctr256, op.stat_out, s); break;
+        case OP_CONV_MFMA256:
+            if (op.deferred) break;
+            e = launch_conv_mfma256(op.conv, op.groups, ctr256, op.stat_out, s); break;
         case OP_CONV64_HALO: e = launch_conv64_halo(op.conv, ctx->n_cus, ticket_ctr(ctx, op), s); break;
         case OP_CONV64S2_HALO: e = launch_conv64s2_halo(op.conv, ctx->n_cus, ticket_ctr(ctx, op), s); break;
         case OP_CONV64_ROOT: e = launch_conv64_root(op.conv, op.root, ctx->n_cus, ticket_ctr(ctx, op), s); break;
@@ -986,7 +1079,10 @@
             break;
         }
         case OP_MAXPOOL: e = launch_maxpool(op.pool, s); break;
-        case OP_SOFTMAX: e = launch_softmax_fuse(op.sm, s); break;
+        case OP_SOFTMAX:
+            e = launch_softmax_fuse(op.sm, s);
+            if (e == hipSuccess && op.fold_conv >= 0) e = launch_conv_mfma256_apply(ctx->ops[op.fold_conv].conv, ctx->ops[op.fold_conv].groups, op.af, ctr256, s);
+            break;
         case OP_PATCH_MASK: e = launch_patch_mask(op.pm, s); break;
         case OP_QUANT_MX8: e = launch_quant_mx8(op.qm, s); break;
         case OP_CONV_MX8: e = launch_conv_mx8(op.cm, op.groups, s); break;
```

Result: faster. 2719, median of 6 (+1.2%).
